# 87003697/DynamiCrafter

Hardware: AMD Instinct MI355X
Metric: frames/sec (and denoising-step ms), 16f@576x1024, DDIM 50 (higher is better)
Workload: dtype bf16; 1 GPU; inference_1024_v1.0.yaml: 1 clip/GPU, 16 frames, latent 72x128, DDIM 50 uniform_trailing eta=1, CFG 7.5 batched (cond+uncond), guidance_rescale 0.7, v-param+ZTSNR+dynamic rescale, hipGraph-captured step; clips_per_gpu=1, parallelism=dp1 over 1 distinct clips (no data-path collective), conditioning=local (1 rank), outputs_finite=True

## Files before the change

### dynamicrafter_amd/_hip.py

```python
import ctypes as C
import os
import threading

_HERE = os.path.dirname(os.path.abspath(__file__))
LIB_PATH = os.environ.get("DC_HIP_LIB") or os.path.join(_HERE, "csrc", "libdcrafter_hip.so")

DC_GEMM_OUT_F32 = 1
DC_GEMM_GEGLU = 2
DC_GEMM_GELU = 4


class DcGemmParams(C.Structure):
    _fields_ = [
        ("A", C.c_void_p), ("W", C.c_void_p), ("C", C.c_void_p), ("bias", C.c_void_p),
        ("rowvec", C.c_void_p), ("residual", C.c_void_p),
        ("lda", C.c_int), ("ldc", C.c_int), ("ldr", C.c_int), ("rowvec_ld", C.c_int),
        ("rows_per_vec", C.c_int),
        ("M", C.c_int), ("N", C.c_int), ("K", C.c_int), ("n_pad", C.c_int),
        ("mode", C.c_int), ("Cin", C.c_int),
        ("IH", C.c_int), ("IW", C.c_int), ("OH", C.c_int), ("OW", C.c_int),
        ("stride", C.c_int), ("pad", C.c_int), ("ups", C.c_int),
        ("T", C.c_int), ("HW", C.c_int),
        ("flags", C.c_int), ("alpha", C.c_float),
        ("workspace", C.c_void_p), ("workspace_bytes", C.c_longlong),
    ]


class DcDdimParams(C.Structure):
    _fields_ = [
        ("a_t", C.c_void_p), ("a_prev", C.c_void_p), ("sigma_t", C.c_void_p), ("sqrt_one_minus_at", C.c_void_p),
        ("sqrt_acp_t", C.c_void_p), ("sqrt_1macp_t", C.c_void_p), ("scale_ratio", C.c_void_p),
        ("step_index", C.c_void_p),
        ("index", C.c_int), ("v_param", C.c_int),
        ("cfg_scale", C.c_float), ("cfg_img", C.c_float), ("guidance_rescale", C.c_float),
        ("temperature", C.c_float),
        ("e_nchw", C.c_int), ("noise_step_stride", C.c_int64),
    ]


class DcDpmParams(C.Structure):
    _fields_ = [
        ("A", C.c_void_p), ("alpha_t", C.c_void_p), ("alpha_p_r", C.c_void_p), ("k", C.c_void_p), ("N", C.c_void_p),
        ("sqrt_one_minus_at", C.c_void_p), ("sqrt_acp_t", C.c_void_p), ("sqrt_1macp_t", C.c_void_p),
        ("scale_ratio", C.c_void_p), ("step_index", C.c_void_p),
        ("index", C.c_int), ("v_param", C.c_int),
        ("cfg_scale", C.c_float), ("cfg_img", C.c_float), ("guidance_rescale", C.c_float),
        ("temperature", C.c_float),
        ("e_nchw", C.c_int), ("noise_step_stride", C.c_int64), ("x0_hist", C.c_void_p),
    ]


class DcSdsParams(C.Structure):
    _fields_ = [
        ("c1", C.c_void_p), ("c2", C.c_void_p), ("w", C.c_void_p), ("step_size", C.c_void_p), ("bc2_sqrt", C.c_void_p),
        ("step_index", C.c_void_p), ("index", C.c_int), ("weight_type", C.c_int), ("x0_param", C.c_int),
        ("e_nchw", C.c_int), ("cfg_scale", C.c_float), ("guidance_rescale", C.c_float),
        ("beta2", C.c_float), ("eps", C.c_float), ("one_minus_beta1", C.c_float), ("one_minus_beta2", C.c_float),
        ("decay", C.c_float), ("grad_scale", C.c_float), ("noise_step_stride", C.c_int64), ("loss", C.c_void_p),
    ]


_P, _I, _F, _L = C.c_void_p, C.c_int, C.c_float, C.c_int64
SIGNATURES = {
    "dc_gemm_conv": (_I, [C.POINTER(DcGemmParams), _P]),
    "dc_gemm_workspace_bytes": (_L, []),
    "dc_gemm_last_variant": (C.c_char_p, []),
    "dc_gemm_set_plan": (_I, [_I]),
    "dc_groupnorm": (_I, [_P, _I, _P, _I, _P, _P, _I, _I, _I, _I, _F, _I, _P, _P]),
    "dc_groupnorm_workspace_bytes": (_L, [_I, _I, _I]),
    "dc_layernorm": (_I, [_P, _I, _P, _I, _P, _P, _I, _I, _F, _P]),
    "dc_flash_attn_d64": (_I, [_P, _P, _P, _P, _I, _I, _I, _I, _I, _I, _I, _I, _L, _L, _F, _I, _F, _P]),
    "dc_ff_geglu_fused320": (_I, [_P, _I, _P, _P, _F, _P, _P, _P, _P, _P, _I, _P, _I, _I, _P]),
    "dc_ff_geglu_proj_fused320": (_I, [_P, _I, _P, _P, _F, _P, _P, _P, _P, _P, _P, _P, _I, _P, _I, _I, _P]),
    "dc_ln_linear": (_I, [_P, _I, _I, _P, _P, _F, _P, _P, _P, _I, _I, _I, _P]),
    "dc_ln_qkv_temporal_attn320": (_I, [_P, _I, _P, _P, _F, _P, _P, _I, _I, _I, _I, _F, _P]),
    "dc_ln_qkv_temporal_attn640": (_I, [_P, _I, _P, _P, _F, _P, _P, _I, _I, _I, _I, _F, _P]),
    "dc_gn_silu_tconv3": (_I, [_P, _I, _I, _P, _P, _P, _I, _P, _P, _P, _I, _P, _I, _I, _I, _I, _I, _P]),
    "dc_groupnorm_stats": (_I, [_P, _I, _I, _I, _I, _I, _F, _P, _P, _P]),
    "dc_gn_linear": (_I, [_P, _I, _I, _P, _P, _P, _I, _I, _P, _P, _P, _I, _I, _I, _P]),
    "dc_flash_attn_set_mode": (_I, [_I, _F]),
    "dc_linear_residual": (_I, [_P, _I, _I, _P, _P, _P, _I, _P, _I, _I, _I, _P]),
    "dc_cross_attn_dual_d64": (_I, [_P, _P, _P, _P, _P, _P, _I, _I, _I, _I, _I, _I, _I, _I, _L, _L, _F, _F, _P]),
    "dc_temporal_attn_d64": (_I, [_P, _I, _P, _I, _I, _I, _I, _I, _F, _P]),
    "dc_gemv_small": (_I, [_P, _I, _P, _P, _P, _I, _I, _I, _I, _I, _I, _I, _P]),
    "dc_timestep_embedding": (_I, [_P, _P, _I, _P, _I, _I, _F, _P]),
    "dc_pack_latent": (_I, [_P, _P, _P, _I, _I, _I, _I, _I, _I, _I, _P]),
    "dc_nchw_to_rows": (_I, [_P, _P, _I, _I, _I, _I, _F, _P]),
    "dc_rows_to_nchw": (_I, [_P, _I, _I, _P, _I, _I, _I, _F, _P]),
    "dc_im2col3x3_c8": (_I, [_P, _I, _P, _I, _I, _I, _I, _P]),
    "dc_copy2d": (_I, [_P, _I, _P, _I, _I, _I, _P]),
    "dc_build_context": (_I, [_P, _P, _I, _I, _I, _I, _I, _P]),
    "dc_softmax_rows": (_I, [_P, _I, _P, _I, _I, _I, _P]),
    "dc_transpose": (_I, [_P, _I, _P, _I, _I, _I, _P]),
    "dc_add_rows": (_I, [_P, _I, _P, _I, _P, _I, _I, _I, _P]),
    "dc_vae_sample": (_I, [_P, _I, _P, _P, _I, _I, _I, _F, _P]),
    "dc_ddim_step": (_I, [C.POINTER(DcDdimParams), _P, _P, _P, _I, _P, _P, _P, _P, _I, _I, _I, _P, _P]),
    "dc_dpmpp_step": (_I, [C.POINTER(DcDpmParams), _P, _P, _P, _I, _P, _P, _P, _P, _I, _I, _I, _P, _P]),
    "dc_sds_noise": (_I, [C.POINTER(DcSdsParams), _P, _P, _P, _I, _L, _P]),
    "dc_sds_step": (_I, [C.POINTER(DcSdsParams), _P, _P, _I, _P, _P, _P, _P, _I, _I, _I, _P, _P]),
    "dc_attn_small": (_I, [_P, _P, _P, _P, _I, _I, _I, _I, _I, _I, _I, _I, _I, _F, _I, _P]),
    "dc_attn_small_lds_bytes": (_L, [_I, _I]),
    "dc_clip_preprocess": (_I, [_P, _P, _P, _P, _I, _I, _I, _I, _I, _I, _I, C.POINTER(_F), C.POINTER(_F), _P]),
    "dc_patchify": (_I, [_P, _P, _I, _I, _I, _I, _I, _I, _P]),
    "dc_embed_tokens": (_I, [_P, _P, _P, _P, _I, _I, _I, _I, _P]),
    "dc_frames_to_u8": (_I, [_P, _P, _I, _I, _I, _I, _I, _P]),
    "dc_mask_blend": (_I, [_P, _P, _P, _P, _P, _P, _P, _I, _L, _L, _I, _P]),
    "dc_advance_counter": (_I, [_P, _P]),
    "dc_stream_create": (_I, [C.POINTER(_P)]),
    "dc_stream_destroy": (_I, [_P]),
    "dc_stream_sync": (_I, [_P]),
    "dc_graph_begin_capture": (_I, [_P]),
    "dc_graph_end_capture": (_I, [_P, C.POINTER(_P)]),
    "dc_graph_launch": (_I, [_P, _P]),
    "dc_graph_destroy": (_I, [_P]),
    "dc_event_create": (_I, [C.POINTER(_P)]),
    "dc_event_record": (_I, [_P, _P]),
    "dc_event_elapsed_ms": (_I, [_P, _P, C.POINTER(_F)]),
    "dc_event_destroy": (_I, [_P]),
    "dc_error_word_read": (_I, [C.POINTER(C.c_int), _I]),
    "dc_version": (C.c_char_p, []),
}

_lib = None
_lock = threading.Lock()


def lib():
    global _lib
    if _lib is not None:
        return _lib
    with _lock:
        if _lib is None:
            if not os.path.exists(LIB_PATH):
                raise RuntimeError(
                    f"{LIB_PATH} not found: build it with dynamicrafter_amd/csrc/build.sh "
                    "(or __graft_entry__.build()); the HIP extension is mandatory, there is no fallback")
            import torch
            l = C.CDLL(LIB_PATH)
            for name, (res, args) in SIGNATURES.items():
                fn = getattr(l, name)
                fn.restype = res
                fn.argtypes = args
            _lib = l
    return _lib


ERROR_WORD_BITS = {1: "gemm_pipe320x16_kernel: LDS counter wait timed out",
                   2: "flash_attn_d64_pipe_kernel: K/V ring counter wait timed out",
                   4: "gemm_pp_kernel: LDS counter wait timed out"}


def check_error_word(what="", reset=True):
    w = C.c_int(0)
    check(lib().dc_error_word_read(C.byref(w), 1 if reset else 0), "dc_error_word_read")
    if w.value:
        names = [v for k, v in ERROR_WORD_BITS.items() if w.value & k] or [f"unknown bits {w.value:#x}"]
        raise RuntimeError(f"HIP kernels reported a failed wait ({what or 'error word'} = {w.value:#x}): " + "; ".join(names)
                           + " - results since the last check are NOT valid")


def check(code, what):
    if code != 0:
        raise RuntimeError(f"{what} failed with code {code}"
                           + (" (DC_ERR_SHAPE)" if code == -1 else " (DC_ERR_ARG)" if code == -2 else " (hipError_t)"))
```

### dynamicrafter_amd/csrc/gemm_conv.hip

```cpp
#include "dc_common.h"
#include "dcrafter_hip.h"
#include <stdlib.h>

namespace {

constexpr int BM = 128;
constexpr int BK = 64;
constexpr int NTHREADS = 256;

__device__ __forceinline__ int lds_off(int row, int chunk) {
    return row * 128 + ((chunk ^ ((row >> 1) & 7)) << 4);
}

__device__ __attribute__((aligned(16))) uint32_t g_zero_chunk[8];

template <int BN, bool GEGLU, int MODE>
__global__ __launch_bounds__(NTHREADS) void gemm_conv_kernel(const DcGemmParams p) {
    constexpr int NB = BN / 64;
    constexpr int BNOUT = GEGLU ? BN / 2 : BN;
    constexpr int A_BYTES = BM * BK * 2;
    constexpr int B_BYTES = BN * BK * 2;
    constexpr int STAGE = A_BYTES + B_BYTES;
    constexpr int B_ITERS = BN / 32;
    extern __shared__ __attribute__((aligned(16))) char smem[];
// ... 228 lines not shown
int launch_mode(const DcGemmParams& p, hipStream_t stream) {
    constexpr int BNOUT = GEGLU ? BN / 2 : BN;
    const int n_out = GEGLU ? p.N / 2 : p.N;
    const int tiles_n = (n_out + BNOUT - 1) / BNOUT;
    const int tiles_m = (p.M + BM - 1) / BM;
    const size_t lds = 2 * (BM * BK * 2 + BN * BK * 2);
    dc_note_variant(GEGLU ? "gemm_conv_kernel<geglu>" : (BN == 64 ? "gemm_conv_kernel<64>" : "gemm_conv_kernel<128>"));
    hipLaunchKernelGGL((gemm_conv_kernel<BN, GEGLU, MODE>), dim3(tiles_m * tiles_n), dim3(NTHREADS), lds, stream, p);
    DC_CHECK_LAUNCH();
    return 0;
}

template <int BN, bool GEGLU>
int launch(const DcGemmParams& p, hipStream_t stream) {
    if (p.mode == 0) return launch_mode<BN, GEGLU, 0>(p, stream);
    if (GEGLU) return DC_ERR_ARG;
    if (p.mode == 1) return launch_mode<BN, false, 1>(p, stream);
    if (p.mode == 2) return launch_mode<BN, false, 2>(p, stream);
    return DC_ERR_ARG;
}


constexpr int NC_TH = 4, NC_TW = 64;
constexpr int NC_WIN_W = NC_TW + 2, NC_WIN = (NC_TH + 2) * NC_WIN_W;
constexpr int NC_LDS = NC_WIN * 128;

__device__ __forceinline__ int nc_off(int px, int chunk) { return px * 128 + ((chunk ^ (px & 7)) << 4); }

template <bool F32>
__global__ __launch_bounds__(256) void conv3x3_narrow_kernel(const DcGemmParams p, const int tiles_x, const int tiles_y) {
    __shared__ __attribute__((aligned(16))) char win[NC_LDS];
    const int tid = threadIdx.x, lane = tid & 63;
    const int wave = __builtin_amdgcn_readfirstlane(tid >> 6);
    const int lj = lane & 15, lq = lane >> 4;
    const int per_frame = tiles_x * tiles_y;
    const int frame = (int)blockIdx.x / per_frame;
    const int trem = (int)blockIdx.x - frame * per_frame;
    const int ty0 = (trem / tiles_x) * NC_TH, tx0 = (trem % tiles_x) * NC_TW;
    const uint16_t* const fbase = p.A + (size_t)frame * p.IH * p.IW * p.lda;

    f32x4_t acc[NC_TW / 16];
#pragma unroll
    for (int b = 0; b < NC_TW / 16; ++b) acc[b] = f32x4_t{0.f, 0.f, 0.f, 0.f};

    const int nslices = p.Cin / 64;
    for (int sl = 0; sl < nslices; ++sl) {
        bf16x8_t wf[9][2];
        {
            const uint16_t* wrow = p.W + (size_t)lj * p.K + (size_t)sl * 576 + lq * 8;
#pragma unroll
            for (int t = 0; t < 9; ++t)
#pragma unroll
                for (int ks = 0; ks < 2; ++ks) {
                    u32x4_t v = {0u, 0u, 0u, 0u};
                    if (lj < p.N) v = *reinterpret_cast<const u32x4_t*>(wrow + t * 64 + ks * 32);
                    wf[t][ks] = __builtin_bit_cast(bf16x8_t, v);
                }
        }
        if (sl > 0) __syncthreads();
        constexpr int NC_IT = (NC_WIN * 8 + 255) / 256;
        u32x4_t stg[NC_IT];
#pragma unroll
        for (int it = 0; it < NC_IT; ++it) {
            int i = tid + it * 256;
            if (i >= NC_WIN * 8) i = NC_WIN * 8 - 1;
            const int px = i >> 3, ch = i & 7;
            const int wy = px / NC_WIN_W, wx = px - wy * NC_WIN_W;
            const int iy = ty0 + wy - 1, ix = tx0 + wx - 1;
            const bool in = iy >= 0 && iy < p.IH && ix >= 0 && ix < p.IW;
            const uint16_t* src = in ? fbase + ((size_t)iy * p.IW + ix) * p.lda + sl * 64 + ch * 8
                                     : reinterpret_cast<const uint16_t*>(g_zero_chunk);
            stg[it] = *reinterpret_cast<const u32x4_t*>(src);
        }
#pragma unroll
        for (int it = 0; it < NC_IT; ++it) {
            const int i = tid + it * 256;
            if (i < NC_WIN * 8) *reinterpret_cast<u32x4_t*>(win + nc_off(i >> 3, i & 7)) = stg[it];
        }
        __syncthreads();
#pragma unroll
        for (int t = 0; t < 9; ++t) {
            const int dy = t / 3, dx = t - 3 * dy;
#pragma unroll
            for (int ks = 0; ks < 2; ++ks)
#pragma unroll
                for (int b = 0; b < NC_TW / 16; ++b) {
                    const int px = (wave + dy) * NC_WIN_W + 16 * b + lj + dx;
                    const bf16x8_t xfrag = *reinterpret_cast<const bf16x8_t*>(win + nc_off(px, ks * 4 + lq));
                    acc[b] = __builtin_amdgcn_mfma_f32_16x16x32_bf16(wf[t][ks], xfrag, acc[b], 0, 0, 0);
                }
        }
    }
    const int oy = ty0 + wave;
    if (oy >= p.IH || 4 * lq >= p.N) return;
    float4 bv = make_float4(0.f, 0.f, 0.f, 0.f);
    if (p.bias) bv = *reinterpret_cast<const float4*>(p.bias + 4 * lq);
#pragma unroll
    for (int b = 0; b < NC_TW / 16; ++b) {
        const int ox = tx0 + 16 * b + lj;
        if (ox >= p.IW) continue;
        const size_t row = ((size_t)frame * p.IH + oy) * p.IW + ox;
        const float v0 = (acc[b][0] + bv.x) * p.alpha, v1 = (acc[b][1] + bv.y) * p.alpha;
        const float v2 = (acc[b][2] + bv.z) * p.alpha, v3 = (acc[b][3] + bv.w) * p.alpha;
        if constexpr (F32) {
            *reinterpret_cast<float4*>(reinterpret_cast<float*>(p.C) + row * p.ldc + 4 * lq) = make_float4(v0, v1, v2, v3);
        } else {
            uint2 pk;
            pk.x = pack_bf2(v0, v1); pk.y = pack_bf2(v2, v3);
            *reinterpret_cast<uint2*>(reinterpret_cast<uint16_t*>(p.C) + row * p.ldc + 4 * lq) = pk;
        }
    }
}

constexpr int WC_N = 128, WC_CB = WC_N / 16;
constexpr int WC_WST = WC_N * 128;
constexpr int NC_GROUPS = (NC_WIN + 7) / 8;
constexpr int WC_WIN_BYTES = NC_GROUPS * 1024;
constexpr int WC_LDS = WC_WIN_BYTES + WC_WST;

__global__ __launch_bounds__(256, 2) void conv3x3_window128_kernel(const DcGemmParams p, const int tiles_x, const int tiles_y) {
    extern __shared__ __attribute__((aligned(16))) char wsm[];
    char* const win = wsm;
    char* const wst = wsm + WC_WIN_BYTES;
    const unsigned lds_base = (unsigned)(uintptr_t)((const __attribute__((address_space(3))) char*)wsm);
    const int tid = threadIdx.x, lane = tid & 63;
    const int wave = __builtin_amdgcn_readfirstlane(tid >> 6);
    const int lj = lane & 15, lq = lane >> 4;
    const int per_frame = tiles_x * tiles_y;
    const int frame = (int)blockIdx.x / per_frame;
    const int trem = (int)blockIdx.x - frame * per_frame;
    const int ty0 = (trem / tiles_x) * NC_TH, tx0 = (trem % tiles_x) * NC_TW;
    const uint16_t* const fbase = p.A + (size_t)frame * p.IH * p.IW * p.lda;

    f32x4_t acc[NC_TW / 16][WC_CB];
#pragma unroll
    for (int b = 0; b < NC_TW / 16; ++b)
#pragma unroll
        for (int c = 0; c < WC_CB; ++c) acc[b][c] = f32x4_t{0.f, 0.f, 0.f, 0.f};

    u32x4_t wreg[4];
    auto w_fetch = [&](int sl, int t) __attribute__((always_inline)) {
#pragma unroll
        for (int i = 0; i < 4; ++i) {
            const int pc = tid + 256 * i;
            wreg[i] = *reinterpret_cast<const u32x4_t*>(p.W + (size_t)(pc >> 3) * p.K + (size_t)sl * 576 + t * 64 + (pc & 7) * 8);
        }
    };
    auto w_store = [&]() __attribute__((always_inline)) {
#pragma unroll
        for (int i = 0; i < 4; ++i) {
            const int pc = tid + 256 * i;
            *reinterpret_cast<u32x4_t*>(wst + nc_off(pc >> 3, pc & 7)) = wreg[i];
        }
    };

    const int nslices = p.Cin / 64;
    w_fetch(0, 0);
#pragma unroll 1
    for (int sl = 0; sl < nslices; ++sl) {
        if (sl > 0) __syncthreads();
        for (int g = wave; g < NC_GROUPS; g += 4) {
            const int px = g * 8 + (lane >> 3), ch = (lane & 7) ^ (px & 7);
            const int wy = px / NC_WIN_W, wx = px - wy * NC_WIN_W;
            const int iy = ty0 + wy - 1, ix = tx0 + wx - 1;
            const bool in = px < NC_WIN && iy >= 0 && iy < p.IH && ix >= 0 && ix < p.IW;
            const uint16_t* src = in ? fbase + ((size_t)iy * p.IW + ix) * p.lda + sl * 64 + ch * 8
                                     : reinterpret_cast<const uint16_t*>(g_zero_chunk);
            asm volatile("s_mov_b32 m0, %1\n\ts_nop 0\n\tglobal_load_lds_dwordx4 %0, off" ::"v"(src), "s"(lds_base + g * 1024) : "memory");
        }
        w_store();
        asm volatile("s_waitcnt vmcnt(0)" ::: "memory");
        __syncthreads();
#pragma unroll 1
        for (int t = 0; t < 9; ++t) {
            if (t + 1 < 9) w_fetch(sl, t + 1);
            else if (sl + 1 < nslices) w_fetch(sl + 1, 0);
            const int dy = t / 3, dx = t - 3 * dy;
#pragma unroll
            for (int ks = 0; ks < 2; ++ks) {
                bf16x8_t xb[NC_TW / 16];
#pragma unroll
                for (int b = 0; b < NC_TW / 16; ++b) {
                    const int px = (wave + dy) * NC_WIN_W + 16 * b + lj + dx;
                    xb[b] = *reinterpret_cast<const bf16x8_t*>(win + nc_off(px, ks * 4 + lq));
                }
#pragma unroll
                for (int c = 0; c < WC_CB; ++c) {
                    const bf16x8_t wa = *reinterpret_cast<const bf16x8_t*>(wst + nc_off(c * 16 + lj, ks * 4 + lq));
#pragma unroll
                    for (int b = 0; b < NC_TW / 16; ++b)
                        acc[b][c] = __builtin_amdgcn_mfma_f32_16x16x32_bf16(wa, xb[b], acc[b][c], 0, 0, 0);
                }
            }
            if (t + 1 < 9) {
                __syncthreads();
                w_store();
                __syncthreads();
            }
        }
    }
    __syncthreads();
    const int oy = ty0 + wave;
    if (oy >= p.IH) return;
    char* const patch = wsm + wave * 8192;
    uint16_t* const cbase = reinterpret_cast<uint16_t*>(p.C);
    const int rpx = lane >> 3, rch = lane & 7;
    const size_t row0 = ((size_t)frame * p.IH + oy) * p.IW + tx0;
#pragma unroll
    for (int hf = 0; hf < 2; ++hf) {
        u32x4_t rres[8];
        if (p.residual) {
#pragma unroll
            for (int it = 0; it < 8; ++it) {
                int px = it * 8 + rpx;
                if (tx0 + px >= p.IW) px = 0;
                rres[it] = *reinterpret_cast<const u32x4_t*>(p.residual + (row0 + px) * p.ldr + hf * 64 + rch * 8);
            }
        }
#pragma unroll
        for (int b = 0; b < NC_TW / 16; ++b)
#pragma unroll
            for (int c4 = 0; c4 < 4; ++c4) {
                const int c = hf * 4 + c4;
                float4 v = make_float4(acc[b][c][0], acc[b][c][1], acc[b][c][2], acc[b][c][3]);
                if (p.bias) {
                    const float4 bv = *reinterpret_cast<const float4*>(p.bias + 16 * c + 4 * lq);
                    v.x += bv.x; v.y += bv.y; v.z += bv.z; v.w += bv.w;
                }
                uint2 pk;
                pk.x = pack_bf2(v.x, v.y); pk.y = pack_bf2(v.z, v.w);
                const int px = 16 * b + lj;
                *reinterpret_cast<uint2*>(patch + nc_off(px, 2 * c4 + (lq >> 1)) + (lq & 1) * 8) = pk;
            }
#pragma unroll
        for (int it = 0; it < 8; ++it) {
            const int px = it * 8 + rpx;
            u32x4_t d = *reinterpret_cast<const u32x4_t*>(patch + nc_off(px, rch));
            if (p.residual) {
#pragma unroll
                for (int e = 0; e < 4; ++e)
                    d[e] = pack_bf2(__uint_as_float(d[e] << 16) + __uint_as_float(rres[it][e] << 16),
                                    __uint_as_float(d[e] & 0xffff0000u) + __uint_as_float(rres[it][e] & 0xffff0000u));
            }
            if (tx0 + px < p.IW) *reinterpret_cast<u32x4_t*>(cbase + (row0 + px) * p.ldc + hf * 64 + rch * 8) = d;
        }
    }
}

inline bool window128_conv_ok(const DcGemmParams& p) {
    if ((dc_gemm_plan_now() & 256) || p.mode != 1 || (p.N != WC_N && p.N != 2 * WC_N) || p.stride != 1 || p.pad != 1 || p.ups) return false;
    if (p.OH != p.IH || p.OW != p.IW || p.Cin % 64 != 0 || p.K != 9 * p.Cin || p.n_pad < p.N) return false;
    if (p.rowvec || p.flags || p.alpha != 1.0f) return false;
    if (p.M % (p.IH * p.IW) != 0 || ((uintptr_t)p.A % 16) != 0 || ((uintptr_t)p.W % 16) != 0 || ((uintptr_t)p.C % 8) != 0) return false;
    if (p.ldc % 8 != 0 || ((uintptr_t)p.C % 16) != 0 || (p.residual && (p.ldr % 8 != 0 || ((uintptr_t)p.residual % 16) != 0))) return false;
    const long long tiles = (long long)(p.M / (p.IH * p.IW)) * ((p.IW + NC_TW - 1) / NC_TW) * ((p.IH + NC_TH - 1) / NC_TH);
    return tiles >= 1024;
}

int launch_window128_conv(const DcGemmParams& p, hipStream_t stream) {
    static DcLdsOnce lds_once;
    if (const int e = lds_once.ensure(reinterpret_cast<const void*>(&conv3x3_window128_kernel), WC_LDS)) return e;
    const int tiles_x = (p.IW + NC_TW - 1) / NC_TW, tiles_y = (p.IH + NC_TH - 1) / NC_TH;
    const long long grid = (long long)(p.M / (p.IH * p.IW)) * tiles_x * tiles_y;
    if (grid <= 0 || grid > 0x7fffffffll) return DC_ERR_SHAPE;
    dc_note_variant(p.N == WC_N ? "conv3x3_window128_kernel" : "conv3x3_window128_kernel x2");
    for (int h = 0; h < p.N / WC_N; ++h) {
        DcGemmParams q = p;
        q.W = p.W + (size_t)h * WC_N * p.K;
        if (p.bias) q.bias = p.bias + h * WC_N;
        q.C = reinterpret_cast<uint16_t*>(p.C) + h * WC_N;
        if (p.residual) q.residual = p.residual + h * WC_N;
        q.N = WC_N;
        hipLaunchKernelGGL(conv3x3_window128_kernel, dim3((unsigned)grid), dim3(256), WC_LDS, stream, q, tiles_x, tiles_y);
        DC_CHECK_LAUNCH();
    }
    return 0;
}

inline bool narrow_conv_ok(const DcGemmParams& p) {
    if ((dc_gemm_plan_now() & 128) || p.mode != 1 || p.N > 16 || p.N % 4 != 0 || p.stride != 1 || p.pad != 1 || p.ups) return false;
    if (p.OH != p.IH || p.OW != p.IW || p.Cin % 64 != 0 || p.K != 9 * p.Cin) return false;
    if (p.residual || p.rowvec || (p.flags & ~DC_GEMM_OUT_F32)) return false;
    if (p.M % (p.IH * p.IW) != 0 || ((uintptr_t)p.A % 16) != 0 || ((uintptr_t)p.W % 16) != 0) return false;
    if ((p.flags & DC_GEMM_OUT_F32) ? ((uintptr_t)p.C % 16 != 0) : (((uintptr_t)p.C % 8) != 0)) return false;
    return true;
}

int launch_narrow_conv(const DcGemmParams& p, hipStream_t stream) {
    const int tiles_x = (p.IW + NC_TW - 1) / NC_TW, tiles_y = (p.IH + NC_TH - 1) / NC_TH;
    const long long grid = (long long)(p.M / (p.IH * p.IW)) * tiles_x * tiles_y;
    if (grid <= 0 || grid > 0x7fffffffll) return DC_ERR_SHAPE;
    dc_note_variant("conv3x3_narrow_kernel");
    if (p.flags & DC_GEMM_OUT_F32)
        hipLaunchKernelGGL(conv3x3_narrow_kernel<true>, dim3((unsigned)grid), dim3(256), 0, stream, p, tiles_x, tiles_y);
    else
        hipLaunchKernelGGL(conv3x3_narrow_kernel<false>, dim3((unsigned)grid), dim3(256), 0, stream, p, tiles_x, tiles_y);
    DC_CHECK_LAUNCH();
    return 0;
}

}

int dc_gemm_conv_glds_try(const DcGemmParams& p, hipStream_t stream);

static bool glds_enabled() {
    static int v = -1;
    if (v < 0) {
        const char* e = getenv("DC_GEMM_GLDS");
        v = (e && e[0] == '0') ? 0 : 1;
    }
    return v == 1;
}

static thread_local const char* g_last_variant = "none";
void dc_note_variant(const char* name) { g_last_variant = name; }
extern "C" const char* dc_gemm_last_variant(void) { return g_last_variant; }

extern "C" int64_t dc_gemm_workspace_bytes(void) {
    return (int64_t)8 * 40 * 256 * 320 * 4;
}

extern "C" int dc_gemm_conv(const DcGemmParams* pp, void* stream_) {
    const DcGemmParams& p = *pp;
    hipStream_t stream = (hipStream_t)stream_;
    if (p.M <= 0 || p.N <= 0 || p.K <= 0) return DC_ERR_SHAPE;
    if (p.K % BK != 0 || p.N % 4 != 0 || p.lda % 8 != 0 || p.ldc % 4 != 0) return DC_ERR_SHAPE;
    if (p.mode != 0 && (p.Cin % BK != 0)) return DC_ERR_SHAPE;
    if (p.mode == 1 && p.K != 9 * p.Cin) return DC_ERR_SHAPE;
    if (p.mode == 2 && p.K != 3 * p.Cin) return DC_ERR_SHAPE;
    if (p.residual && (p.ldr % 4 != 0)) return DC_ERR_SHAPE;
    const bool geglu = (p.flags & DC_GEMM_GEGLU) != 0;
    if (geglu && ((p.N / 2) % 64 != 0 || p.n_pad < p.N)) return DC_ERR_SHAPE;
    if (p.n_pad < (p.N + 127) / 128 * 128) return DC_ERR_SHAPE;
    if (narrow_conv_ok(p)) return launch_narrow_conv(p, stream);
    if (window128_conv_ok(p)) return launch_window128_conv(p, stream);
    if (glds_enabled()) {
        const int r = dc_gemm_conv_glds_try(p, stream);
        if (r != -100) return r;
    }
    if (geglu) return launch<128, true>(p, stream);
    const int t128 = (p.N + 127) / 128 * 128;
    const bool use64 = (p.N <= 64) || ((float)t128 / (float)p.N > 1.15f);
    if (use64) {
        if (p.n_pad < (p.N + 63) / 64 * 64) return DC_ERR_SHAPE;
        return launch<64, false>(p, stream);
    }
    if (p.n_pad < t128) return DC_ERR_SHAPE;
    return launch<128, false>(p, stream);
}
```

### dynamicrafter_amd/csrc/gemm_conv_glds.hip

```cpp
#include "dc_common.h"
#include "dcrafter_hip.h"
#include <stdint.h>
#include <stdlib.h>
#include <type_traits>
#include <utility>

namespace {

constexpr int GBM = 256;
constexpr int GBK = 64;
constexpr int GNT = 512;

typedef __attribute__((address_space(3))) char lds_char_t;

__device__ __attribute__((aligned(16))) uint32_t g_zero_chunk2[8];

__device__ __forceinline__ int lds_off2(int row, int chunk) {
    return row * 128 + ((chunk ^ ((row >> 1) & 7)) << 4);
}

__device__ __forceinline__ void glds16(const void* gsrc, unsigned lds_dst_uniform) {
    unsigned keep;
    asm volatile(
        "s_mov_b32 %0, m0\n\t"
// ... 526 lines not shown

    const unsigned lds_base = (unsigned)(unsigned long)((lds_char_t*)smem);
    const bf16_t* const zero_ptr = reinterpret_cast<const bf16_t*>(g_zero_chunk2);
    const int srow = lane >> 3;
    const int pchunk = lane & 7;

    const bf16_t* a_ptr[A_IT];
    int a_aux[A_IT];
    const bf16_t* b_ptr[B_IT];
    int i_tile = 0, i_kt = 0, i_stage = 0;
    int i_m0 = 0, i_n0 = 0;
    auto set_issue_tile = [&](int j) __attribute__((always_inline)) {
        const int logical = xcd_remap((int)blockIdx.x + j * G, ntiles);
        int tn, tmi;
        persist_tile(logical, tiles_m, tiles_n, tile_group, tmi, tn);
        const int m0 = tmi * GBM, n0 = tn * BNOUT;
        i_m0 = m0; i_n0 = n0;
#pragma unroll
        for (int q = 0; q < A_IT; ++q) {
            const int r = (q * 8 + wave) * 8 + srow;
            const int chunk = pchunk ^ ((r >> 1) & 7);
            const int m = m0 + r;
            const bool ok = m < p.M;
            a_aux[q] = 0;
            if (MODE == 0) {
                a_ptr[q] = ok ? p.A + (size_t)m * p.lda + chunk * 8 : nullptr;
            } else if (MODE == 1) {
                const int ohw = p.OH * p.OW;
                const int mm = ok ? m : 0;
                const int n = mm / ohw;
                const int rem = mm - n * ohw;
                const int oy = rem / p.OW;
                const int ox = rem - oy * p.OW;
                const int iy0 = oy * p.stride - p.pad, ix0 = ox * p.stride - p.pad;
                int mask = 0;
#pragma unroll
                for (int t = 0; t < 9; ++t) {
                    const int iy = iy0 + t / 3, ix = ix0 + t % 3;
                    if (ok && iy >= 0 && iy < p.IH && ix >= 0 && ix < p.IW) mask |= 1 << t;
                }
                a_aux[q] = mask;
                a_ptr[q] = p.A + ((long long)n * p.IH * p.IW + (long long)iy0 * p.IW + ix0) * p.lda + chunk * 8;
            } else {
                a_ptr[q] = p.A + (size_t)(ok ? m : 0) * p.lda + chunk * 8;
                a_aux[q] = ok ? (m / p.HW) % p.T : -1000;
            }
        }
#pragma unroll
        for (int q = 0; q < B_IT; ++q) {
            const int r = (q * 8 + wave) * 8 + srow;
            const int chunk = pchunk ^ ((r >> 1) & 7);
            int wrow;
            if (GEGLU) wrow = (r < BN / 2) ? (n0 + r) : ((p.N >> 1) + n0 + (r - BN / 2));
            else wrow = n0 + r;
            b_ptr[q] = p.W + (size_t)wrow * p.K + chunk * 8;
        }
    };
    auto issue_next_part = [&](int part) __attribute__((always_inline)) {
        const int k0 = i_kt * GBK;
        const unsigned sa = lds_base + i_stage * STAGE;
        const unsigned sb = sa + A_BYTES;
        const bool res_tile = RES_RING && i_kt >= nk;
#pragma unroll
        for (int q = 0; q < A_IT; ++q) {
            if (q != part) continue;
            const bf16_t* src;
            if (res_tile) {
                const int r = (q * 8 + wave) * 8 + srow;
                const int chunk = pchunk ^ ((r >> 1) & 7);
                const int m = i_m0 + r;
                const int col = i_n0 + (i_kt - nk) * 32 + (chunk >> 2) * (BN / 2) + (chunk & 3) * 8;
                src = (m < p.M) ? p.residual + (size_t)m * p.ldr + col : zero_ptr;
            } else if (MODE == 0) {
                src = a_ptr[q] ? a_ptr[q] + k0 : zero_ptr;
            } else if (MODE == 1) {
                const int cs = i_kt / 9;
                const int tap = i_kt - cs * 9;
                const int dy = tap / 3, dx = tap - dy * 3;
                const long long toff = (long long)(dy * p.IW + dx) * p.lda + cs * 64;
                src = ((a_aux[q] >> tap) & 1) ? a_ptr[q] + toff : zero_ptr;
            } else {
                const int cs = i_kt / 3;
                const int tap = i_kt - cs * 3;
                const long long shift = (long long)(tap - 1) * p.HW * p.lda + cs * 64;
                const int tt = a_aux[q] + tap - 1;
                src = (tt >= 0 && tt < p.T) ? a_ptr[q] + shift : zero_ptr;
            }
            glds16(src, sa + (q * 8 + wave) * 1024);
        }
        if (!res_tile) {
#pragma unroll
            for (int q = 0; q < B_IT; ++q)
                if ((q & 3) == part) glds16(b_ptr[q] + k0, sb + (q * 8 + wave) * 1024);
        }
        if (part == 3) {
            if (++i_stage >= GSTAGES) i_stage = 0;
            if (++i_kt >= nkr) {
                i_kt = 0;
                ++i_tile;
                if (i_tile < nj) set_issue_tile(i_tile);
            }
        }
    };
    auto issue_next = [&]() __attribute__((always_inline)) {
#pragma unroll
        for (int part = 0; part < 4; ++part) issue_next_part(part);
    };

    f32x16_t acc[2][NB];
    auto zero_acc = [&]() __attribute__((always_inline)) {
#pragma unroll
        for (int i = 0; i < 2; ++i)
#pragma unroll
            for (int j = 0; j < NB; ++j)
#pragma unroll
                for (int r = 0; r < 16; ++r) acc[i][j][r] = 0.f;
    };
    zero_acc();

    set_issue_tile(0);
    issue_next();
    if (GSTAGES >= 3 && total > 1) issue_next();
    if (GSTAGES == 4 && total > 2) issue_next();

    int c_tile = 0, c_kt = 0, stage = 0;
    for (int g = 0; g < total; ++g) {
        const int younger = total - 1 - g;
        if (GSTAGES == 4 && younger >= 2) {
            static_assert(GSTAGES != 4 || !RES_RING, "4-deep ring: residual tiles not counted");
            wait_vmcnt<2 * LOADS>();
        } else if (GSTAGES >= 3 && younger >= 1) {
            if (RES_RING && c_kt + 1 >= nk) wait_vmcnt<A_IT>(); else wait_vmcnt<LOADS>();
        } else {
            wait_vmcnt<0>();
        }
        __builtin_amdgcn_s_barrier();
        asm volatile("" ::: "memory");
        const bool more = g + GSTAGES - 1 < total;
        const char* sa = smem + stage * STAGE;
        const char* sb = sa + A_BYTES;
        {
#pragma unroll
            for (int kk = 0; kk < GBK / 16; ++kk) {
                if (more) issue_next_part(kk);
                bf16x8_t xf[2], wf[NB];
#pragma unroll
                for (int mb = 0; mb < 2; ++mb)
                    xf[mb] = *reinterpret_cast<const bf16x8_t*>(sa + lds_off2(wm * 64 + mb * 32 + fr, kk * 2 + fh));
#pragma unroll
                for (int nb = 0; nb < NB; ++nb) {
                    int brow;
                    if (GEGLU) brow = (nb < NBX ? 0 : BN / 2) + wn * (BN / 4) + (nb % NBX) * 32;
                    else brow = wn * (32 * NB) + nb * 32;
                    wf[nb] = *reinterpret_cast<const bf16x8_t*>(sb + lds_off2(brow + fr, kk * 2 + fh));
                }
#pragma unroll
                for (int mb = 0; mb < 2; ++mb)
#pragma unroll
                    for (int nb = 0; nb < NB; ++nb)
                        acc[mb][nb] = __builtin_amdgcn_mfma_f32_32x32x16_bf16(wf[nb], xf[mb], acc[mb][nb], 0, 0, 0);
            }
        }
        if (++stage >= GSTAGES) stage = 0;
        if (++c_kt >= nk) {
            if constexpr (RES_RING) {
#pragma unroll
                for (int j = 0; j < NB; ++j) {
                    ++g;
                    const int younger_r = total - 1 - g;
                    if (GSTAGES >= 3 && younger_r >= 1) {
                        if (j + 1 < NB) wait_vmcnt<A_IT>(); else wait_vmcnt<LOADS>();
                    } else {
                        wait_vmcnt<0>();
                    }
                    __builtin_amdgcn_s_barrier();
                    asm volatile("" ::: "memory");
                    if (g + GSTAGES - 1 < total) {
#pragma unroll
                        for (int kk = 0; kk < GBK / 16; ++kk) issue_next_part(kk);
                    }
                    const char* sr = smem + stage * STAGE;
                    int lane_r = lane;
                    asm volatile("" : "+v"(lane_r));
                    const int fr_r = lane_r & 31, fh_r = lane_r >> 5;
#pragma unroll
                    for (int i = 0; i < 2; ++i) {
                        const int e1 = fr_r - 16 * i - 8 * fh_r;
                        bf16x8_t idf;
#pragma unroll
                        for (int e = 0; e < 8; ++e) idf[e] = (e == e1) ? (short)0x3F80 : (short)0;
#pragma unroll
                        for (int mb = 0; mb < 2; ++mb) {
                            const bf16x8_t xr = *reinterpret_cast<const bf16x8_t*>(
                                sr + lds_off2(wm * 64 + mb * 32 + fr_r, (wn * 2 + i) * 2 + fh_r));
                            acc[mb][j] = __builtin_amdgcn_mfma_f32_32x32x16_bf16(idf, xr, acc[mb][j], 0, 0, 0);
                        }
                    }
                    if (++stage >= GSTAGES) stage = 0;
                }
            }
            c_kt = 0;
            const int logical = xcd_remap((int)blockIdx.x + c_tile * G, ntiles);
            ++c_tile;
            int tn, tmi;
            persist_tile(logical, tiles_m, tiles_n, tile_group, tmi, tn);
            const int m0 = tmi * GBM, n0 = tn * BNOUT;
            persist_epilogue<BN, GEGLU, EPI>(acc, p, m0, n0, n_out, wm, wn, lane, smem + GSTAGES * STAGE + wave * 2048);
            zero_acc();
        }
    }
}

template <int BN, bool GEGLU, int EPI, int MODE, int ST_FORCE>
int launch_persist_epi_st(const DcGemmParams& p, hipStream_t stream, int grid);

template <int BN, bool GEGLU, int EPI, int MODE>
int launch_persist_epi(const DcGemmParams& p, hipStream_t stream, int grid) {
    static const int st = [] { const char* e = getenv("DC_GEMM_STAGES"); return e ? atoi(e) : 0; }();
    if constexpr (BN <= 128 && MODE == 0 && !GEGLU) { if (st == 2) return launch_persist_epi_st<BN, GEGLU, EPI, MODE, 2>(p, stream, grid); }
    return launch_persist_epi_st<BN, GEGLU, EPI, MODE, 0>(p, stream, grid);
}

template <int BN, bool GEGLU, int EPI, int MODE, int ST_FORCE>
int launch_persist_epi_st(const DcGemmParams& p, hipStream_t stream, int grid) {
    constexpr int ST = ST_FORCE ? ST_FORCE : ((BN <= 128) ? 3 : 2);
    constexpr size_t lds = (size_t)ST * (GBM * GBK * 2 + BN * GBK * 2) + 8 * 2048;
    static_assert(lds <= 163840, "LDS budget");
    static DcLdsOnce lds_once;
    if (const int e = lds_once.ensure(reinterpret_cast<const void*>(&gemm_persist_kernel<BN, GEGLU, ST, EPI, MODE>), (int)lds)) return e;
    dc_note_variant(GEGLU ? (BN == 256 ? "gemm_persist_kernel<256,geglu>" : "gemm_persist_kernel<128,geglu>")
                    : MODE == 1 ? "gemm_persist_kernel<320,conv>" : MODE == 2 ? "gemm_persist_kernel<320,tconv>"
                    : BN == 320 ? (EPI == 1 || EPI == 3 ? "gemm_persist_kernel<320,residual>" : "gemm_persist_kernel<320>")
                    : BN == 128 ? "gemm_persist_kernel<128>" : "gemm_persist_kernel<64>");
    static const int group = [] { const char* e = getenv("DC_GEMM_GROUP"); return e ? atoi(e) : 8; }();
    hipLaunchKernelGGL((gemm_persist_kernel<BN, GEGLU, ST, EPI, MODE>), dim3(grid), dim3(GNT), lds, stream, p,
                       (group == 2 || group == 4 || group == 8 || group == 16) ? group : 1);
    DC_CHECK_LAUNCH();
    return 0;
}

inline bool ring_residual_ok(const DcGemmParams& p) {
    static const int on = [] { const char* e = getenv("DC_GEMM_RING_RESIDUAL"); return e ? atoi(e) : 1; }();
    return on && p.residual && !(p.flags & (DC_GEMM_GELU | DC_GEMM_GEGLU | DC_GEMM_OUT_F32)) && p.alpha == 1.0f &&
           (p.N % 64 == 0) && (p.ldr % 8 == 0) && ((uintptr_t)p.residual % 16 == 0);
}

template <int BN, bool GEGLU>
int launch_persist(const DcGemmParams& p, hipStream_t stream, int grid) {
    if (p.flags & DC_GEMM_OUT_F32) {
        if constexpr (GEGLU) return DC_ERR_ARG;
        else return launch_persist_epi<BN, GEGLU, 2, 0>(p, stream, grid);
    }
    if (p.residual) {
        if constexpr (!GEGLU) { if (ring_residual_ok(p) && p.N % BN == 0) return launch_persist_epi<BN, GEGLU, 3, 0>(p, stream, grid); }
        return launch_persist_epi<BN, GEGLU, 1, 0>(p, stream, grid);
    }
    return launch_persist_epi<BN, GEGLU, 0, 0>(p, stream, grid);
}

int launch_persist_conv320(const DcGemmParams& p, hipStream_t stream) {
    const bool ring = ring_residual_ok(p);
    if (p.mode == 1) return p.residual ? (ring ? launch_persist_epi<320, false, 3, 1>(p, stream, 256)
                                               : launch_persist_epi<320, false, 1, 1>(p, stream, 256))
                                       : launch_persist_epi<320, false, 0, 1>(p, stream, 256);
    return p.residual ? (ring ? launch_persist_epi<320, false, 3, 2>(p, stream, 256)
                              : launch_persist_epi<320, false, 1, 2>(p, stream, 256))
                      : launch_persist_epi<320, false, 0, 2>(p, stream, 256);
}

template <int BN, bool GEGLU, int MODE, int GSTAGES>
int launch_glds(const DcGemmParams& p, hipStream_t stream) {
    constexpr int BNOUT = GEGLU ? BN / 2 : BN;
    const int n_out = GEGLU ? p.N / 2 : p.N;
    const int tiles_n = (n_out + BNOUT - 1) / BNOUT;
    const int tiles_m = (p.M + GBM - 1) / GBM;
    constexpr size_t lds = (size_t)GSTAGES * (GBM * GBK * 2 + BN * GBK * 2);
    static DcLdsOnce lds_once;
    if (const int e = lds_once.ensure(reinterpret_cast<const void*>(&gemm_conv_glds_kernel<BN, GEGLU, MODE, GSTAGES>), (int)lds)) return e;
    GemmSplit sp;
    sp.partial = nullptr; sp.splits = 1; sp.tile_begin = 0; sp.tile_count = tiles_m * tiles_n; sp.err = nullptr; sp.whole = 0;
    dc_note_variant(GEGLU ? "gemm_conv_glds_kernel<geglu>"
                    : BN == 320 ? (MODE == 0 ? "gemm_conv_glds_kernel<320>" : MODE == 2 ? "gemm_conv_glds_kernel<320,tconv>" : "gemm_conv_glds_kernel<320,conv>")
                    : BN == 256 ? (MODE == 0 ? "gemm_conv_glds_kernel<256>" : MODE == 2 ? "gemm_conv_glds_kernel<256,tconv>" : "gemm_conv_glds_kernel<256,conv>")
                    : (MODE == 0 ? "gemm_conv_glds_kernel<128>" : MODE == 2 ? "gemm_conv_glds_kernel<128,tconv>" : "gemm_conv_glds_kernel<128,conv>"));
    hipLaunchKernelGGL((gemm_conv_glds_kernel<BN, GEGLU, MODE, GSTAGES>), dim3(tiles_m * tiles_n), dim3(GNT), lds, stream, p, sp);
    DC_CHECK_LAUNCH();
    return 0;
}

constexpr int PLAN_DEFAULT = 3 | 16;
constexpr int PLAN_MASK = 3 | 16 | 32 | 64 | 128 | 256;
inline bool plan_valid(int plan) { return plan >= 0 && plan <= 511 && !(plan & 4); }
std::atomic<int> g_gemm_plan{[] {
    const char* e = getenv("DC_GEMM_PLAN");
    const int v = e ? atoi(e) : PLAN_DEFAULT;
    return plan_valid(v) ? (v & PLAN_MASK) : PLAN_DEFAULT;
}()};
inline int pipe_min_k() { static const int v = [] { const char* e = getenv("DC_PIPE_MIN_K"); return e ? atoi(e) : 1920; }(); return v; }

template <int MODE, int EPI>
int launch_pipe_shape(const DcGemmParams& p, hipStream_t stream, GemmSplit sp, int gx, int gy) {
    sp.err = dc_error_word_device();
    if (!sp.err) return DC_ERR_ARG;
    return launch_pipe320x16<MODE, EPI>(p, stream, sp, gx, gy);
}

inline bool pipe_ok(const DcGemmParams& p, int plan) {
    if (!(plan & 3) || (!(plan & 2) && p.mode != 1)) return false;
    if (p.mode != 1 && p.K < pipe_min_k()) return false;
    if (p.flags & (DC_GEMM_GEGLU | DC_GEMM_OUT_F32)) return false;
    if (p.ups && !(p.mode == 1 && p.ups == 1 && p.stride == 1 && p.pad == 1 && p.OH == 2 * p.IH && p.OW == 2 * p.IW)) return false;
    if (p.N % 320 != 0 || p.n_pad < p.N || p.K % 64 != 0 || p.lda % 8 != 0 || ((uintptr_t)p.A % 16) != 0) return false;
    if (p.ldc % 8 != 0 || ((uintptr_t)p.C % 16) != 0 || (long long)p.M * p.ldc >= (1ll << 31)) return false;
    if (p.residual && (p.ldr % 8 != 0 || ((uintptr_t)p.residual % 16) != 0 || (long long)p.M * p.ldr >= (1ll << 31))) return false;
    long long rows = p.M, extra = 0;
    if (p.mode == 1) { if (p.Cin % 64 != 0 || p.K != 9 * p.Cin) return false; rows = (long long)(p.M / (p.OH * p.OW) + 1) * p.IH * p.IW; extra = 2ll * p.IW + 2; }
    else if (p.mode == 2) { if (p.Cin % 64 != 0 || p.K != 3 * p.Cin) return false; extra = 2ll * p.HW; }
    else if (p.mode != 0) return false;
    if ((rows + extra) * p.lda * 2 >= (1ll << 31)) return false;
    if (320ll * p.K * 2 >= (1ll << 31)) return false;
    return true;
}

int launch_pipe_whole(const DcGemmParams& p, hipStream_t stream) {
    const int ntiles = ((p.M + GBM - 1) / GBM) * (p.N / 320);
    GemmSplit sp;
    sp.partial = nullptr; sp.splits = 1; sp.tile_begin = 0; sp.tile_count = ntiles; sp.err = nullptr; sp.whole = 0;
    dc_note_variant(p.mode == 0 ? "gemm_pipe320x16_kernel" : p.mode == 2 ? "gemm_pipe320x16_kernel<tconv>"
                    : p.ups ? "gemm_pipe320x16_kernel<conv,ups>" : "gemm_pipe320x16_kernel<conv>");
    if (p.mode == 0) return p.residual ? launch_pipe_shape<0, 1>(p, stream, sp, ntiles, 1) : launch_pipe_shape<0, 0>(p, stream, sp, ntiles, 1);
    if (p.mode == 1 && p.ups) return p.residual ? launch_pipe_shape<3, 1>(p, stream, sp, ntiles, 1) : launch_pipe_shape<3, 0>(p, stream, sp, ntiles, 1);
    if (p.mode == 1) return p.residual ? launch_pipe_shape<1, 1>(p, stream, sp, ntiles, 1) : launch_pipe_shape<1, 0>(p, stream, sp, ntiles, 1);
    return p.residual ? launch_pipe_shape<2, 1>(p, stream, sp, ntiles, 1) : launch_pipe_shape<2, 0>(p, stream, sp, ntiles, 1);
}

template <int MODE, int BN = 320>
int launch_glds320_split(const DcGemmParams& p, hipStream_t stream, int ntiles, int full, int splits, bool use_pipe, bool merged) {
    constexpr int GSTAGES = 2;
    constexpr size_t lds = (size_t)GSTAGES * (GBM * GBK * 2 + BN * GBK * 2);
    static DcLdsOnce lds_once;
    if (const int e = lds_once.ensure(reinterpret_cast<const void*>(&gemm_conv_glds_kernel<BN, false, MODE, GSTAGES>), (int)lds)) return e;
    if constexpr (BN == 320) {
        if (use_pipe) {
            dc_note_variant(MODE == 0 ? "gemm_pipe320x16_kernel+splitk" : MODE == 2 ? "gemm_pipe320x16_kernel<tconv>+splitk"
                            : MODE == 3 ? "gemm_pipe320x16_kernel<conv,ups>+splitk" : "gemm_pipe320x16_kernel<conv>+splitk");
            GemmSplit sp;
            sp.err = nullptr; sp.whole = 0;
            if (full > 0 && merged && full % 8 == 0) {
                sp.partial = reinterpret_cast<float*>(p.workspace); sp.splits = splits; sp.tile_begin = full; sp.tile_count = ntiles - full;
                sp.whole = full;
                const int gx = full + sp.tile_count * splits;
                if (const int e = p.residual ? launch_pipe_shape<MODE, 1>(p, stream, sp, gx, 1) : launch_pipe_shape<MODE, 0>(p, stream, sp, gx, 1)) return e;
                sp.whole = 0;
            } else {
                if (full > 0) {
                    sp.partial = nullptr; sp.splits = 1; sp.tile_begin = 0; sp.tile_count = full;
                    if (const int e = p.residual ? launch_pipe_shape<MODE, 1>(p, stream, sp, full, 1) : launch_pipe_shape<MODE, 0>(p, stream, sp, full, 1)) return e;
                }
                sp.partial = reinterpret_cast<float*>(p.workspace); sp.splits = splits; sp.tile_begin = full; sp.tile_count = ntiles - full;
                if (const int e = launch_pipe_shape<MODE, 0>(p, stream, sp, sp.tile_count, splits)) return e;
            }
            hipLaunchKernelGGL((splitk_reduce_kernel<BN>), dim3((GBM * (BN / 4) + 255) / 256, sp.tile_count), dim3(256), 0, stream, p, sp);
            DC_CHECK_LAUNCH();
            return 0;
        }
    }
    if constexpr (BN == 320)
        dc_note_variant(MODE == 0 ? "gemm_conv_glds_kernel<320>+splitk" : MODE == 2 ? "gemm_conv_glds_kernel<320,tconv>+splitk" : "gemm_conv_glds_kernel<320,conv>+splitk");
    else
        dc_note_variant(MODE == 0 ? "gemm_conv_glds_kernel<256>+splitk" : MODE == 2 ? "gemm_conv_glds_kernel<256,tconv>+splitk" : "gemm_conv_glds_kernel<256,conv>+splitk");
    GemmSplit sp;
    sp.err = nullptr; sp.whole = 0;
    if (full > 0) {
        sp.partial = nullptr; sp.splits = 1; sp.tile_begin = 0; sp.tile_count = full;
        hipLaunchKernelGGL((gemm_conv_glds_kernel<BN, false, MODE, GSTAGES>), dim3(full), dim3(GNT), lds, stream, p, sp);
        DC_CHECK_LAUNCH();
    }
    sp.partial = reinterpret_cast<float*>(p.workspace); sp.splits = splits; sp.tile_begin = full; sp.tile_count = ntiles - full;
    hipLaunchKernelGGL((gemm_conv_glds_kernel<BN, false, MODE, GSTAGES>), dim3(sp.tile_count, splits), dim3(GNT), lds, stream, p, sp);
    DC_CHECK_LAUNCH();
    hipLaunchKernelGGL((splitk_reduce_kernel<BN>), dim3((GBM * (BN / 4) + 255) / 256, sp.tile_count), dim3(256), 0, stream, p, sp);
    DC_CHECK_LAUNCH();
    return 0;
}

template <int BN, int GSTAGES>
int launch_glds_mode(const DcGemmParams& p, hipStream_t stream) {
    if (p.mode == 0) return launch_glds<BN, false, 0, GSTAGES>(p, stream);
    if (p.mode == 1) return p.ups ? launch_glds<BN, false, 3, GSTAGES>(p, stream) : launch_glds<BN, false, 1, GSTAGES>(p, stream);
    return launch_glds<BN, false, 2, GSTAGES>(p, stream);
}

inline int persist_max_k() {
    static const int v = [] { const char* e = getenv("DC_GEMM_PERSIST_MAXK"); return e ? atoi(e) : 2560; }();
    return v;
}

inline float wave_eff(int wgs) { return (float)wgs / (float)(((wgs + 255) / 256) * 256); }

}

int dc_gemm_conv_glds_try(const DcGemmParams& p, hipStream_t stream) {
    const bool geglu = (p.flags & DC_GEMM_GEGLU) != 0;
    const int n_out = geglu ? p.N / 2 : p.N;
    const int tiles_m = (p.M + GBM - 1) / GBM;
    static const int force = [] { const char* e = getenv("DC_GEMM_TILE"); return e ? atoi(e) : 0; }();
    static const int persist = [] { const char* e = getenv("DC_GEMM_PERSIST"); return e ? atoi(e) : 1; }();
    if (geglu && p.mode != 0) return DC_ERR_ARG;
    const bool out_f32 = (p.flags & DC_GEMM_OUT_F32) != 0;
    const bool epi16 = out_f32 || ((n_out % 8 == 0) && (p.ldc % 8 == 0) && ((long long)p.M * p.ldc < (1ll << 31)) &&
                                   ((long long)p.M * p.ldr < (1ll << 31)) && ((uintptr_t)p.C % 16 == 0) &&
                                   (!p.residual || ((p.ldr % 8 == 0) && ((uintptr_t)p.residual % 16 == 0))));
    const int plan = g_gemm_plan.load(std::memory_order_relaxed);
    const bool use_pipe = pipe_ok(p, plan);
    const bool prefer_pipe = (force == 0) && use_pipe;
    if (persist && force == 0 && p.mode == 0 && epi16 && p.K <= persist_max_k() && !prefer_pipe) {
        static const int wide = [] { const char* e = getenv("DC_GEMM_PERSIST_WIDE"); return e ? atoi(e) : 1; }();
        if (geglu && (plan & 16) && ((plan & 32) || p.K <= 640) && pp_ok(p) && tiles_m * (n_out / 64) >= 1024) return launch_pp(p, stream);
        if (geglu) {
            if (wide && n_out % 128 == 0 && tiles_m * (n_out / 128) >= 512) return launch_persist<256, true>(p, stream, 256);
            const int nt = tiles_m * (n_out / 64);
            if (nt >= 512) return launch_persist<128, true>(p, stream, 256);
        } else {
            if (wide && p.N % 320 == 0 && p.n_pad >= p.N && tiles_m * (p.N / 320) >= 512)
                return launch_persist<320, false>(p, stream, 256);
            const int t128n = (p.N + 127) / 128;
            const float waste = (float)(t128n * 128) / (float)p.N;
            if (waste <= 1.15f && tiles_m * t128n >= 512) return launch_persist<128, false>(p, stream, 256);
            const int t64n = (p.N + 63) / 64;
            if (waste > 1.15f && tiles_m * t64n >= 512) return launch_persist<64, false>(p, stream, 256);
        }
    }
    static const int persist_conv_maxk = [] { const char* e = getenv("DC_GEMM_PERSIST_CONV_MAXK"); return e ? atoi(e) : 2880; }();
    if (persist && force == 0 && !prefer_pipe && !geglu && !out_f32 && epi16 && (p.mode == 2 || (p.mode == 1 && !p.ups)) &&
        p.N % 320 == 0 && p.n_pad >= p.N && tiles_m * (p.N / 320) >= (p.mode == 1 ? 1024 : 512) && p.K <= persist_conv_maxk)
        return launch_persist_conv320(p, stream);
    if (geglu) {
        const int w256 = (n_out % 128 == 0 && p.n_pad >= p.N) ? tiles_m * (n_out / 128) : 0;
        const int w128 = tiles_m * (n_out / 64);
        if ((force == 256 || (force == 0 && w256 >= 512 && wave_eff(w256) > 0.8f)) && w256 > 0)
            return launch_glds<256, true, 0, 2>(p, stream);
        if (w128 < 384) return -100;
        return launch_glds<128, true, 0, 3>(p, stream);
    }
    const int t128 = (p.N + 127) / 128;
    const bool n320 = (p.N % 320 == 0) && (p.n_pad >= p.N);
    const int w320 = n320 ? tiles_m * (p.N / 320) : 0;
    const int w128 = tiles_m * t128;
    const float waste128 = (float)(t128 * 128) / (float)p.N;
    const bool pipe_conv = use_pipe && p.mode == 1 && force == 0;
    float s320 = n320 ? (pipe_conv ? 1.4f : 1.25f) * wave_eff(w320) : 0.f;
    float s128 = wave_eff(w128) / waste128;
    if (w320 < (pipe_conv ? 128 : 200)) s320 = 0.f;
    if (w128 < 384) s128 = 0.f;
    static const int splitk = [] { const char* e = getenv("DC_GEMM_SPLITK"); return e ? atoi(e) : 1; }();
    if (splitk && force == 0 && n320 && p.workspace && p.n_pad >= p.N) {
        const int nk = p.K / GBK;
        int full = 0, splits = 0;
        if (w320 < 200 && w320 >= 8) {
            splits = 256 / w320;
            if (splits > 12) splits = 12;
            while (splits > 2 && nk / splits < 12) --splits;
        } else if (w320 > 256 && w320 <= 1280 && (w320 % 256) != 0 && (w320 % 256) <= 128) {
            full = (w320 / 256) * 256;
            splits = 256 / (w320 - full);
            if (splits > 8) splits = 8;
            while (splits > 2 && nk / splits < 8) --splits;
        }
        const size_t need = (size_t)splits * (size_t)(w320 - full) * GBM * 320 * sizeof(float);
        if (splits >= 2 && nk / splits >= (full ? 8 : 12) && need <= (size_t)p.workspace_bytes) {
            const bool merged = !(plan & 64);
            if (p.mode == 0) return launch_glds320_split<0>(p, stream, w320, full, splits, use_pipe, merged);
            if (p.mode == 1) return p.ups ? launch_glds320_split<3>(p, stream, w320, full, splits, use_pipe, merged)
                                          : launch_glds320_split<1>(p, stream, w320, full, splits, use_pipe, merged);
            return launch_glds320_split<2>(p, stream, w320, full, splits, use_pipe, merged);
        }
    }
    static const int splitk256 = [] { const char* e = getenv("DC_GEMM_SPLITK256"); return e ? atoi(e) : 1; }();
    if (splitk && splitk256 && force == 0 && !n320 && !out_f32 && p.workspace && p.N % 256 == 0 && p.n_pad >= p.N && (p.mode != 1 || !p.ups)) {
        const int w256s = tiles_m * (p.N / 256), nk = p.K / GBK;
        if (w256s > 256 && w256s <= 1280 && (w256s % 256) != 0 && (w256s % 256) <= 128) {
            const int full = (w256s / 256) * 256;
            int splits = 256 / (w256s - full);
            if (splits > 8) splits = 8;
            while (splits > 2 && nk / splits < 8) --splits;
            const size_t need = (size_t)splits * (size_t)(w256s - full) * GBM * 256 * sizeof(float);
            if (splits >= 2 && nk / splits >= 8 && need <= (size_t)p.workspace_bytes) {
                if (p.mode == 0) return launch_glds320_split<0, 256>(p, stream, w256s, full, splits, false, false);
                if (p.mode == 1) return launch_glds320_split<1, 256>(p, stream, w256s, full, splits, false, false);
                return launch_glds320_split<2, 256>(p, stream, w256s, full, splits, false, false);
            }
        }
    }
    if (force == 320 && n320) return use_pipe ? launch_pipe_whole(p, stream) : launch_glds_mode<320, 2>(p, stream);
    if (force == 128 && w128 > 0 && waste128 <= 1.15f) return launch_glds_mode<128, 3>(p, stream);
    if (force == 1) return -100;
    const int w256 = (!n320 && p.N % 256 == 0 && p.n_pad >= p.N) ? tiles_m * (p.N / 256) : 0;
    if ((force == 256 || force == 0) && w256 >= 200 && 1.2f * wave_eff(w256) >= s128) return launch_glds_mode<256, 2>(p, stream);
    if (s320 > 0.f && s320 >= s128) return use_pipe ? launch_pipe_whole(p, stream) : launch_glds_mode<320, 2>(p, stream);
    if (s128 > 0.f && waste128 <= 1.15f) return launch_glds_mode<128, 3>(p, stream);
    return -100;
}

int dc_gemm_plan_now() { return g_gemm_plan.load(std::memory_order_relaxed); }

extern "C" int dc_gemm_set_plan(int plan) {
    if (!plan_valid(plan)) return DC_ERR_ARG;
    return g_gemm_plan.exchange(plan & PLAN_MASK, std::memory_order_relaxed);
}
```

### dynamicrafter_amd/csrc/gemm_pipe16.h

```cpp
#pragma once

typedef __attribute__((ext_vector_type(4))) float gp_f32x4_t;

#define GP16_MFMA_A(d, w, x) asm volatile("v_mfma_f32_16x16x32_bf16 %0, %1, %2, %0" : "+a"(d) : "v"(w), "v"(x))
#define GP16_MFMA_V(d, w, x) asm volatile("v_mfma_f32_16x16x32_bf16 %0, %1, %2, %0" : "+v"(d) : "v"(w), "v"(x))

__device__ __forceinline__ void gp16_settle(gp_f32x4_t (&acc)[4][20]) {
#pragma unroll
    for (int rb = 0; rb < 4; ++rb)
        asm volatile("s_nop 7\n\ts_nop 7"
                     : "+a"(acc[rb][0]), "+a"(acc[rb][1]), "+a"(acc[rb][2]), "+a"(acc[rb][3]), "+a"(acc[rb][4]), "+a"(acc[rb][5]),
                       "+a"(acc[rb][6]), "+a"(acc[rb][7]), "+a"(acc[rb][8]), "+a"(acc[rb][9]), "+a"(acc[rb][10]), "+a"(acc[rb][11]),
                       "+a"(acc[rb][12]), "+a"(acc[rb][13]), "+a"(acc[rb][14]), "+a"(acc[rb][15]), "+v"(acc[rb][16]), "+v"(acc[rb][17]),
                       "+v"(acc[rb][18]), "+v"(acc[rb][19]));
    asm volatile("s_nop 7\n\ts_nop 7" ::: "memory");
}

template <int MODE, int EPI>
__global__ __launch_bounds__(256, 1) __attribute__((amdgpu_waves_per_eu(1, 1)))
void gemm_pipe320x16_kernel(const DcGemmParams p, const GemmSplit sp) {
    extern __shared__ __attribute__((aligned(16))) char smem[];
    const int tid = threadIdx.x, lane = tid & 63;
    const int wave = __builtin_amdgcn_readfirstlane(tid >> 6);
    const int lr = lane & 15, lq = lane >> 4;

    const int tiles_n = p.N / 320;
    int bx = blockIdx.x, by = blockIdx.y, tile_begin = sp.tile_begin, tile_count = sp.tile_count, nsplit = sp.splits;
    float* partial = sp.partial;
    if (sp.whole > 0) {
        if (bx < sp.whole) { tile_begin = 0; tile_count = sp.whole; nsplit = 1; partial = nullptr; by = 0; }
        else { bx -= sp.whole; by = bx / tile_count; bx -= by * tile_count; }
    }
    const int swz = tile_begin + xcd_remap(bx, tile_count);
    const int tile_n = swz % tiles_n;
    const int tile_m = swz / tiles_n;
    const int m0 = tile_m * GBM;
    const int n0 = tile_n * 320;

    const int nk_all = p.K / GBK;
    const int kt_lo = (int)(((long long)by * nk_all) / nsplit);
    const int kt_hi = (int)(((long long)(by + 1) * nk_all) / nsplit);
    const int nk = kt_hi - kt_lo;

    gp_lds_int_t* const cnt_landed = (gp_lds_int_t*)(smem + GP_CNT);
    gp_lds_int_t* const cnt_freed = cnt_landed + 1;
    if (tid < 2) cnt_landed[tid] = 0;
    __syncthreads();
    int gave_up = 0;

    const unsigned lda2 = (unsigned)p.lda * 2u;
    unsigned rowoff[4];
    int mask[4];
    long long bias = 0;
    if (MODE == 1) bias = (long long)(p.pad * p.IW + p.pad) * lda2;
    if (MODE == 2) bias = (long long)p.HW * lda2;
    if (MODE == 3) bias = (long long)(p.IW + 1) * lda2;
#ifdef GP_DBG_QUAD_ROWS
    const int lr_a = lr & ~3, lq_a = lane & 3;
#else
    const int lr_a = lr, lq_a = lq;
#endif
#pragma unroll
    for (int rb = 0; rb < 4; ++rb) {
        const int m = m0 + wave * 64 + rb * 16 + lr_a;
        const bool ok = m < p.M;
        const int mm = ok ? m : 0;
        if (MODE == 0) {
            rowoff[rb] = (unsigned)mm * lda2 + lq_a * 16;
            mask[rb] = ok ? 1 : 0;
        } else if (MODE == 1) {
            const int ohw = p.OH * p.OW;
            const int n = mm / ohw;
            const int rem = mm - n * ohw;
            const int oy = rem / p.OW;
            const int ox = rem - oy * p.OW;
            const int iy0 = oy * p.stride - p.pad, ix0 = ox * p.stride - p.pad;
            int mk = 0;
#pragma unroll
            for (int t = 0; t < 9; ++t) {
                const int iy = iy0 + t / 3, ix = ix0 + t % 3;
                if (ok && iy >= 0 && iy < p.IH && ix >= 0 && ix < p.IW) mk |= 1 << t;
            }
            mask[rb] = mk;
            rowoff[rb] = (unsigned)(((n * p.IH + iy0 + p.pad) * p.IW + ix0 + p.pad)) * lda2 + lq_a * 16;
        } else if (MODE == 3) {
            const int ohw = p.OH * p.OW;
            const int n = mm / ohw;
            const int rem = mm - n * ohw;
            const int oy = rem / p.OW;
            const int ox = rem - oy * p.OW;
            int mk = 0;
#pragma unroll
            for (int t = 0; t < 9; ++t) {
                const int uy = oy + t / 3 - 1, ux = ox + t % 3 - 1;
                if (ok && uy >= 0 && uy < p.OH && ux >= 0 && ux < p.OW) mk |= 1 << t;
            }
            mask[rb] = mk | ((oy & 1) << 9) | ((ox & 1) << 10);
            rowoff[rb] = (unsigned)(((n * p.IH + (oy >> 1) + 1) * p.IW + (ox >> 1) + 1)) * lda2 + lq_a * 16;
        } else {
            const int frame = (mm / p.HW) % p.T;
            int mk = 0;
#pragma unroll
            for (int t = 0; t < 3; ++t) {
                const int tt = frame + t - 1;
                if (ok && tt >= 0 && tt < p.T) mk |= 1 << t;
            }
            mask[rb] = mk;
            rowoff[rb] = (unsigned)mm * lda2 + lq_a * 16;
        }
    }
    gp_i32x4_t ars;
    {
        const unsigned long long ab = (unsigned long long)(uintptr_t)p.A - (unsigned long long)bias;
        ars[0] = __builtin_amdgcn_readfirstlane((int)(unsigned)ab);
        ars[1] = __builtin_amdgcn_readfirstlane((int)(unsigned)((ab >> 32) & 0xffffu));
        ars[2] = 0x7fffffff;
        ars[3] = 0x00020000;
    }
    auto a_tile = [&](int kt, unsigned (&vo)[4], int& soff) __attribute__((always_inline)) {
        int tap = 0;
        if (MODE == 0) {
            soff = kt * 128;
        } else if (MODE == 1) {
            const int cs = kt / 9;
            tap = kt - cs * 9;
            const int dy = tap / 3, dx = tap - dy * 3;
            soff = (dy * p.IW + dx) * (int)lda2 + cs * 128;
        } else if (MODE == 3) {
            const int cs = kt / 9;
            tap = kt - cs * 9;
            const int dy = tap / 3, dx = tap - dy * 3;
            soff = cs * 128;
            const int y0 = dy == 0 ? -p.IW * (int)lda2 : 0, y1 = dy == 2 ? p.IW * (int)lda2 : 0;
            const int x0 = dx == 0 ? -(int)lda2 : 0, x1 = dx == 2 ? (int)lda2 : 0;
#pragma unroll
            for (int rb = 0; rb < 4; ++rb) {
                const unsigned o = rowoff[rb] + (unsigned)(((mask[rb] >> 9) & 1) ? y1 : y0) + (unsigned)(((mask[rb] >> 10) & 1) ? x1 : x0);
                vo[rb] = ((mask[rb] >> tap) & 1) ? o : 0x80000000u;
            }
            return;
        } else {
            const int cs = kt / 3;
            tap = kt - cs * 3;
            soff = tap * p.HW * (int)lda2 + cs * 128;
        }
#pragma unroll
        for (int rb = 0; rb < 4; ++rb) vo[rb] = ((mask[rb] >> tap) & 1) ? rowoff[rb] : 0x80000000u;
    };

    const unsigned lds_base = (unsigned)(uintptr_t)((const __attribute__((address_space(3))) char*)smem);
    unsigned voffB[10];
#pragma unroll
    for (int j = 0; j < 10; ++j) {
        const int row = (j * 4 + wave) * 8 + (lane >> 3);
        voffB[j] = (unsigned)row * (unsigned)p.K * 2u + (unsigned)(((lane & 7) ^ (((wave & 1) * 4 + (lane >> 4)) & 7)) << 4);
        asm volatile("" : "+v"(voffB[j]));
    }
    auto w_src = [&](int kt) __attribute__((always_inline)) -> unsigned long long {
        return (unsigned long long)(uintptr_t)p.W + ((unsigned long long)n0 * p.K + (unsigned long long)kt * 64) * 2ull;
    };
    auto dma = [&](unsigned lds_dst, unsigned voff, unsigned long long sbase) __attribute__((always_inline)) {
        asm volatile("s_mov_b32 m0, %0\n\ts_nop 0\n\tglobal_load_lds_dwordx4 %1, %2" ::"s"(lds_dst), "v"(voff), "s"(sbase) : "memory");
    };

    unsigned bofs[3][2];
#pragma unroll
    for (int st = 0; st < 3; ++st)
#pragma unroll
        for (int s = 0; s < 2; ++s) {
            bofs[st][s] = lds_base + st * GP_STAGE + lr * 128 + (((4 * s + lq) ^ ((lr >> 1) & 7)) << 4);
            asm volatile("" : "+v"(bofs[st][s]));
        }
    bf16x8_t Bf[5];
    auto rd_b = [&](int slot, unsigned addr, int cb) __attribute__((always_inline)) {
        Bf[slot] = *(gp_lds_frag_t*)((const __attribute__((address_space(3))) char*)(uintptr_t)addr + cb * 2048);
    };

    u32x4_t A[3][4][2];
    gp_f32x4_t acc[4][20];
#pragma unroll
    for (int i = 0; i < 4; ++i)
#pragma unroll
        for (int j = 0; j < 20; ++j)
#pragma unroll
            for (int r = 0; r < 4; ++r) acc[i][j][r] = 0.f;

    auto clampk = [&](int t) { return kt_lo + (t < nk ? t : nk - 1); };
#pragma unroll
    for (int t = 0; t < 2; ++t) {
        const unsigned long long ws = w_src(clampk(t));
#pragma unroll
        for (int j = 0; j < 10; ++j) dma(lds_base + t * GP_STAGE + (j * 4 + wave) * 1024, voffB[j], ws);
        unsigned vo[4];
        int soff;
        a_tile(clampk(t), vo, soff);
#pragma unroll
        for (int i = 0; i < 8; ++i) {
            if ((i >> 2) == 0) GP_LOAD_A_(A[t][i & 3][0], vo[i & 3], ars, soff, "0");
            else GP_LOAD_A_(A[t][i & 3][1], vo[i & 3], ars, soff, "64");
        }
    }
    wait_vmcnt<26>();
    if (lane == 0) __hip_atomic_fetch_add(cnt_landed, 1, __ATOMIC_RELAXED, __HIP_MEMORY_SCOPE_WORKGROUP);
    {
        int seen = *(volatile gp_lds_int_t*)cnt_landed;
        GP_SPIN(__builtin_amdgcn_readfirstlane(seen) < 4, seen = *(volatile gp_lds_int_t*)cnt_landed);
        asm volatile("" ::: "memory");
    }
#pragma unroll
    for (int f = 0; f < 4; ++f) rd_b(f, bofs[0][0], f);
    gp16_settle(acc);

    int seen_f = 0, seen_l = 0;
    auto tile = [&](auto ST_, int t) __attribute__((always_inline)) {
        constexpr int ST = decltype(ST_)::value, ST1 = (ST + 1) % 3, ST2 = (ST + 2) % 3;
        const int kt2 = clampk(t + 2);
        unsigned vo[4] = {0u, 0u, 0u, 0u};
        int soff = 0;
        unsigned long long ws = 0;
        gp_f32x4_t (&acc1)[4][20] = acc;
        bf16x8_t (&Bf1)[5] = Bf;
        u32x4_t (&A1)[3][4][2] = A;
        gp_for(std::make_integer_sequence<int, 160>{}, [&](auto G_) __attribute__((always_inline)) {
            constexpr int g = decltype(G_)::value;
            gp_f32x4_t (&acc_)[4][20] = acc1;
            bf16x8_t (&Bf_)[5] = Bf1;
            u32x4_t (&A_)[3][4][2] = A1;
            if constexpr (g == 0) {
                wait_vmcnt<18>();
#pragma unroll
                for (int i = 0; i < 8; ++i) asm volatile("" : "+v"(A_[ST][i & 3][i >> 2]));
            }
            if constexpr ((g & 3) == 0) {
                constexpr int F = g / 4 + 4;
                if constexpr (F < 40) rd_b(F % 5, bofs[ST][F / 20], F % 20);
                else rd_b(F % 5, bofs[ST1][0], F - 40);
            } else if constexpr ((g & 3) == 2) {
                if constexpr (g == 2) seen_f = *(volatile gp_lds_int_t*)cnt_freed;
                if constexpr (g == 6) {
                    GP_SPIN(__builtin_amdgcn_readfirstlane(seen_f) < 4 * t, seen_f = *(volatile gp_lds_int_t*)cnt_freed);
                    asm volatile("" ::: "memory");
                    ws = w_src(kt2);
                }
                if constexpr (g >= 10 && g <= 82 && ((g - 10) & 7) == 0) {
                    constexpr int j = (g - 10) >> 3;
                    dma(lds_base + ST2 * GP_STAGE + (j * 4 + wave) * 1024, voffB[j], ws);
                }
                if constexpr (g == 86) {
                    wait_vmcnt<18>();
#ifdef GP_DBG_SKIP_POST
                    if (lane == 0 && !(wave == 3 && t == 1))
#else
                    if (lane == 0)
#endif
                        __hip_atomic_fetch_add(cnt_landed, 1, __ATOMIC_RELAXED, __HIP_MEMORY_SCOPE_WORKGROUP);
                    a_tile(kt2, vo, soff);
                }
                if constexpr (g >= 90 && g <= 146 && ((g - 90) & 7) == 0) {
                    constexpr int i = (g - 90) >> 3;
                    if constexpr ((i >> 2) == 0) GP_LOAD_A_(A_[ST2][i & 3][0], vo[i & 3], ars, soff, "0");
                    else GP_LOAD_A_(A_[ST2][i & 3][1], vo[i & 3], ars, soff, "64");
                }
                if constexpr (g == 118) seen_l = *(volatile gp_lds_int_t*)cnt_landed;
                if constexpr (g == 142) {
                    GP_SPIN(t + 1 < nk && __builtin_amdgcn_readfirstlane(seen_l) < 4 * (t + 2), seen_l = *(volatile gp_lds_int_t*)cnt_landed);
                    asm volatile("" ::: "memory");
                }
                if constexpr (g == 150) {
                    if (lane == 0) __hip_atomic_fetch_add(cnt_freed, 1, __ATOMIC_RELAXED, __HIP_MEMORY_SCOPE_WORKGROUP);
                }
            }
            constexpr int f = g / 4, rb = g & 3, s = f / 20, cb = f % 20;
            if constexpr (cb < 16) GP16_MFMA_A(acc_[rb][cb], Bf_[f % 5], A_[ST][rb][s]);
            else GP16_MFMA_V(acc_[rb][cb], Bf_[f % 5], A_[ST][rb][s]);
        });
    };
#ifdef GP_STAMPS
    const unsigned long long st_loop0 = __builtin_readcyclecounter();
    const unsigned long long st_real0 = __builtin_amdgcn_s_memrealtime();
#endif
    for (int t = 0; t < nk; t += 3) {
        tile(gp_ic<0>{}, t);
        if (t + 1 >= nk) break;
        tile(gp_ic<1>{}, t + 1);
        if (t + 2 >= nk) break;
        tile(gp_ic<2>{}, t + 2);
    }
    wait_vmcnt<0>();
    gp16_settle(acc);
    if (gave_up && lane == 0) atomicOr(sp.err, DC_ERRW_GEMM_PIPE);
#ifdef GP_STAMPS
    if (lane == 0 && p.workspace && !sp.partial && (size_t)(blockIdx.x * 4 + wave + 1) * 64 <= (size_t)p.workspace_bytes) {
        unsigned long long* out = reinterpret_cast<unsigned long long*>(p.workspace) + (size_t)(blockIdx.x * 4 + wave) * 8;
        out[0] = 0; out[1] = 0; out[2] = 0; out[3] = 0;
        out[4] = __builtin_readcyclecounter() - st_loop0; out[5] = (unsigned long long)nk;
        out[6] = __builtin_amdgcn_s_memrealtime() - st_real0;
    }
#endif

    if (partial) {
        const size_t slot = (size_t)by * tile_count + (size_t)(swz - tile_begin);
        float* const dst = partial + (slot * GBM + wave * 64 + lr) * 320 + 4 * lq;
#pragma unroll
        for (int rb = 0; rb < 4; ++rb)
#pragma unroll
            for (int cb = 0; cb < 20; ++cb)
                *reinterpret_cast<float4*>(dst + (size_t)rb * 16 * 320 + cb * 16) = make_float4(acc[rb][cb][0], acc[rb][cb][1], acc[rb][cb][2], acc[rb][cb][3]);
        return;
    }
    char* const ebuf = smem + GP_RING + wave * 2048;
    int lane_e = lane;
    asm volatile("" : "+v"(lane_e));
    const int er = lane_e & 15, eq = lane_e >> 4;
    const int rrow = lane_e >> 2, rc = lane_e & 3;
    const char* const rbase = reinterpret_cast<const char*>(p.residual);
    char* const cbase = reinterpret_cast<char*>(p.C);
#pragma unroll
    for (int rb = 0; rb < 4; ++rb) {
        const int m_acc = m0 + wave * 64 + rb * 16 + er;
        const float* rv = p.rowvec ? p.rowvec + (size_t)((m_acc < p.M ? m_acc : 0) / p.rows_per_vec) * p.rowvec_ld : nullptr;
        int mr = m0 + wave * 64 + rb * 16 + rrow;
        const bool rok = mr < p.M;
        if (!rok) mr = p.M - 1;
        const unsigned co = ((unsigned)mr * (unsigned)p.ldc + (unsigned)(n0 + rc * 8)) * 2u;
        const unsigned ro = ((unsigned)mr * (unsigned)p.ldr + (unsigned)(n0 + rc * 8)) * 2u;
#pragma unroll
        for (int cp = 0; cp < 10; ++cp) {
            u32x4_t rr;
            if constexpr (EPI == 1) rr = *reinterpret_cast<const u32x4_t*>(rbase + ro + cp * 64);
#pragma unroll
            for (int h = 0; h < 2; ++h) {
                const int cb = 2 * cp + h;
                const int n = n0 + cb * 16 + 4 * eq;
                float4 v = make_float4(acc[rb][cb][0], acc[rb][cb][1], acc[rb][cb][2], acc[rb][cb][3]);
                if (p.bias) {
                    const float4 bv = *reinterpret_cast<const float4*>(p.bias + n);
                    v.x += bv.x; v.y += bv.y; v.z += bv.z; v.w += bv.w;
                }
                if (p.flags & DC_GEMM_GELU) { v.x = DC_GELU(v.x); v.y = DC_GELU(v.y); v.z = DC_GELU(v.z); v.w = DC_GELU(v.w); }
                if (rv) {
                    const float4 r4 = *reinterpret_cast<const float4*>(rv + n);
                    v.x += r4.x; v.y += r4.y; v.z += r4.z; v.w += r4.w;
                }
                if (p.alpha != 1.0f) { v.x *= p.alpha; v.y *= p.alpha; v.z *= p.alpha; v.w *= p.alpha; }
                uint2 pk;
                pk.x = pack_bf2(v.x, v.y);
                pk.y = pack_bf2(v.z, v.w);
                *reinterpret_cast<uint2*>(ebuf + er * 64 + ((((4 * h + eq) ^ (((er >> 1) & 3) << 1))) << 3)) = pk;
            }
            u32x4_t d = *reinterpret_cast<const u32x4_t*>(ebuf + rrow * 64 + ((rc ^ ((rrow >> 1) & 3)) << 4));
            if constexpr (EPI == 1) {
#pragma unroll
                for (int e = 0; e < 4; ++e)
                    d[e] = pack_bf2(__uint_as_float(d[e] << 16) + __uint_as_float(rr[e] << 16),
                                    __uint_as_float(d[e] & 0xffff0000u) + __uint_as_float(rr[e] & 0xffff0000u));
            }
            if (rok) *reinterpret_cast<u32x4_t*>(cbase + co + cp * 64) = d;
            __builtin_amdgcn_sched_barrier(0);
        }
    }
}

template <int MODE, int EPI>
int launch_pipe320x16(const DcGemmParams& p, hipStream_t stream, const GemmSplit& sp, int grid_x, int grid_y) {
    static DcLdsOnce lds_once;
    if (const int e = lds_once.ensure(reinterpret_cast<const void*>(&gemm_pipe320x16_kernel<MODE, EPI>), GP_LDS)) return e;
    hipLaunchKernelGGL((gemm_pipe320x16_kernel<MODE, EPI>), dim3(grid_x, grid_y), dim3(256), GP_LDS, stream, p, sp);
    DC_CHECK_LAUNCH();
    return 0;
}
```

### dynamicrafter_amd/lvdm/modules/networks/openaimodel3d.py

```python
import math

import torch
import torch.nn as nn

from .... import ops
from ....ops import PackedWeight
from ....param_tree import attach_params

import os

_BF16 = torch.bfloat16
_FF_FUSED = os.environ.get("DC_FF_FUSED", "1") != "0"
_LN_FUSED = os.environ.get("DC_LN_FUSED", "1") != "0"
_LR_FUSED = os.environ.get("DC_LR_FUSED", "1") != "0"
_TA_FUSED = os.environ.get("DC_TA_FUSED", "1") != "0"
_TA_FUSED_C = tuple(int(k) for k in os.environ.get("DC_TA_FUSED_C", "320,640").split(","))
_FFP_FUSED = os.environ.get("DC_FFP_FUSED", "1") != "0"
_TC_FUSED = os.environ.get("DC_TC_FUSED", "1") != "0"
_FUSED_MIN_ROWS = int(os.environ.get("DC_FUSED_MIN_ROWS", "4096"))
_LN_FUSED_K = tuple(int(k) for k in os.environ.get("DC_LN_FUSED_K", "320,640").split(","))
C_IN_PAD = 64


def _block_layout(cfg):
    mc, mults, nrb = cfg["model_channels"], list(cfg["channel_mult"]), cfg["num_res_blocks"]
    attn_res = set(cfg["attention_resolutions"])
    hc = cfg["num_head_channels"]
    tconv = bool(cfg["temporal_conv"])

    def transformers(ch):
        out = [("spatial", {"ch": ch, "heads": ch // hc})]
        if cfg["temporal_attention"]:
            out.append(("temporal", {"ch": ch, "inner": ch, "heads": ch // hc, "linear": bool(cfg["use_linear"])}))
        return out

    down_path = [[("conv_in", {"cin": cfg["in_channels"], "cout": mc})]]
    widths = [mc]
    ch, ds = mc, 1
    for lvl, m in enumerate(mults):
        for _ in range(nrb):
            blk = [("res", {"cin": ch, "cout": m * mc, "tconv": tconv})]
            ch = m * mc
            if ds in attn_res:
                blk += transformers(ch)
            down_path.append(blk)
            widths.append(ch)
        if lvl + 1 < len(mults):
            down_path.append([("down", {"ch": ch})])
            widths.append(ch)
            ds *= 2
    middle = [("res", {"cin": ch, "cout": ch, "tconv": tconv})] + transformers(ch) + \
             [("res", {"cin": ch, "cout": ch, "tconv": tconv})]
    up_path = []
    for lvl in reversed(range(len(mults))):
        for i in range(nrb + 1):
            skip = widths.pop()
            blk = [("res", {"cin": ch + skip, "cout": mults[lvl] * mc, "tconv": tconv})]
            ch = mults[lvl] * mc
            if ds in attn_res:
                blk += transformers(ch)
            if lvl and i == nrb:
                blk.append(("up", {"ch": ch}))
                ds //= 2
            up_path.append(blk)
    return down_path, middle, up_path


def _shape_table(cfg):
    t = {}
    mc = cfg["model_channels"]
    emb_dim = 4 * mc

    def affine(p, c):
        t[p + ".weight"] = (c,)
        t[p + ".bias"] = (c,)

    def dense(p, i, o, bias=True):
        t[p + ".weight"] = (o, i)
        if bias:
            t[p + ".bias"] = (o,)

    def conv(p, i, o, *k):
        t[p + ".weight"] = (o, i) + tuple(k)
        t[p + ".bias"] = (o,)

    def attn(p, dim, ctx, with_ip):
        dense(p + ".to_q", dim, dim, False)
        dense(p + ".to_k", ctx, dim, False)
        dense(p + ".to_v", ctx, dim, False)
        dense(p + ".to_out.0", dim, dim)
        if with_ip:
            dense(p + ".to_k_ip", ctx, dim, False)
            dense(p + ".to_v_ip", ctx, dim, False)
            if cfg["image_cross_attention_scale_learnable"]:
                t[p + ".alpha"] = ()

    def tblock(p, dim, ctx, with_ip):
        attn(p + ".attn1", dim, dim, False)
        dense(p + ".ff.net.0.proj", dim, 8 * dim)
        dense(p + ".ff.net.2", 4 * dim, dim)
        attn(p + ".attn2", dim, ctx, with_ip)
        for n in ("norm1", "norm2", "norm3"):
            affine(f"{p}.{n}", dim)

    def temporal(p, ch, inner, linear):
        affine(p + ".norm", ch)
        if linear:
            dense(p + ".proj_in", ch, inner)
        else:
            conv(p + ".proj_in", ch, inner, 1)
        tblock(p + ".transformer_blocks.0", inner, inner, False)
        if linear:
            dense(p + ".proj_out", inner, ch)
        else:
            conv(p + ".proj_out", inner, ch, 1)

    dense("time_embed.0", mc, emb_dim)
    dense("time_embed.2", emb_dim, emb_dim)
    if cfg["fs_condition"]:
        dense("fps_embedding.0", mc, emb_dim)
        dense("fps_embedding.2", emb_dim, emb_dim)

    def emit(prefix, blk):
        for j, (kind, a) in enumerate(blk):
            p = f"{prefix}.{j}"
            if kind == "conv_in":
                conv(p, a["cin"], a["cout"], 3, 3)
            elif kind == "res":
                affine(p + ".in_layers.0", a["cin"])
                conv(p + ".in_layers.2", a["cin"], a["cout"], 3, 3)
                dense(p + ".emb_layers.1", emb_dim, a["cout"])
                affine(p + ".out_layers.0", a["cout"])
                conv(p + ".out_layers.3", a["cout"], a["cout"], 3, 3)
                if a["cin"] != a["cout"]:
                    conv(p + ".skip_connection", a["cin"], a["cout"], 1, 1)
                if a["tconv"]:
                    for i, ci in ((1, 2), (2, 3), (3, 3), (4, 3)):
                        affine(f"{p}.temopral_conv.conv{i}.0", a["cout"])
                        conv(f"{p}.temopral_conv.conv{i}.{ci}", a["cout"], a["cout"], 3, 1, 1)
            elif kind == "spatial":
                affine(p + ".norm", a["ch"])
                dense(p + ".proj_in", a["ch"], a["ch"])
                tblock(p + ".transformer_blocks.0", a["ch"], cfg["context_dim"], bool(cfg["image_cross_attention"]))
                dense(p + ".proj_out", a["ch"], a["ch"])
            elif kind == "temporal":
                temporal(p, a["ch"], a["inner"], a["linear"])
            elif kind == "down":
                conv(p + ".op", a["ch"], a["ch"], 3, 3)
            elif kind == "up":
                conv(p + ".conv", a["ch"], a["ch"], 3, 3)

    down_path, middle, up_path = _block_layout(cfg)
    emit("input_blocks.0", down_path[0])
    if cfg["addition_attention"]:
        temporal("init_attn.0", mc, 8 * cfg["num_head_channels"], False)
    for i, blk in enumerate(down_path[1:], start=1):
        emit(f"input_blocks.{i}", blk)
    emit("middle_block", middle)
    for i, blk in enumerate(up_path):
        emit(f"output_blocks.{i}", blk)
    affine("out.0", mc)
    conv("out.2", mc, cfg["out_channels"], 3, 3)
    return t


_Arena = ops.Arena


class UNetModel(nn.Module):
    def __init__(self, in_channels, model_channels, out_channels, num_res_blocks, attention_resolutions,
                 dropout=0.0, channel_mult=(1, 2, 4, 8), conv_resample=True, dims=2, context_dim=None,
                 use_scale_shift_norm=False, resblock_updown=False, num_heads=-1, num_head_channels=-1,
                 transformer_depth=1, use_linear=False, use_checkpoint=False, temporal_conv=False,
                 tempspatial_aware=False, temporal_attention=True, use_relative_position=True,
                 use_causal_attention=False, temporal_length=None, use_fp16=False, addition_attention=False,
                 temporal_selfatt_only=True, image_cross_attention=False,
                 image_cross_attention_scale_learnable=False, default_fs=4, fs_condition=False):
        super().__init__()
        unsupported = []
        if dims != 2: unsupported.append("dims != 2")
        if use_scale_shift_norm: unsupported.append("use_scale_shift_norm")
        if resblock_updown: unsupported.append("resblock_updown")
        if not conv_resample: unsupported.append("conv_resample=False")
        if num_head_channels != 64: unsupported.append("num_head_channels != 64 (kernels are head_dim 64)")
        if transformer_depth != 1: unsupported.append("transformer_depth != 1")
        if not use_linear: unsupported.append("use_linear=False")
        if tempspatial_aware: unsupported.append("tempspatial_aware")
        if use_relative_position: unsupported.append("use_relative_position")
        if use_causal_attention: unsupported.append("use_causal_attention")
        if not temporal_selfatt_only: unsupported.append("temporal cross-attention")
        if context_dim is None: unsupported.append("context_dim=None")
        if temporal_length is not None and temporal_length > 16: unsupported.append("temporal_length > 16")
        if model_channels % 64 != 0: unsupported.append("model_channels % 64 != 0")
        if unsupported:
            raise NotImplementedError("UNetModel (HIP path) covers the released DynamiCrafter configurations; "
                                      "unsupported here: " + ", ".join(unsupported))
        self.in_channels, self.model_channels, self.out_channels = in_channels, model_channels, out_channels
        self.num_res_blocks = num_res_blocks
        self.attention_resolutions = list(attention_resolutions)
        self.channel_mult = list(channel_mult)
        self.dropout, self.use_checkpoint = dropout, use_checkpoint
        self.temporal_attention, self.temporal_length = temporal_attention, temporal_length
        self.addition_attention = addition_attention
        self.image_cross_attention = image_cross_attention
        self.image_cross_attention_scale_learnable = image_cross_attention_scale_learnable
        self.default_fs, self.fs_condition = default_fs, fs_condition
        self.context_dim = context_dim
        self.dtype = torch.float32
        self._cfg = dict(in_channels=in_channels, out_channels=out_channels, model_channels=model_channels,
                         attention_resolutions=list(attention_resolutions), num_res_blocks=num_res_blocks,
                         channel_mult=list(channel_mult), num_head_channels=num_head_channels,
                         context_dim=context_dim, temporal_conv=temporal_conv, temporal_attention=temporal_attention,
                         addition_attention=addition_attention, image_cross_attention=image_cross_attention,
                         image_cross_attention_scale_learnable=image_cross_attention_scale_learnable,
                         fs_condition=fs_condition, use_linear=use_linear)
        self._layout = _block_layout(self._cfg)
        self._cat_plan = self._make_cat_plan()
        attach_params(self, _shape_table(self._cfg))
        self._packed = None
        self._arena = _Arena()
        self.register_load_state_dict_post_hook(lambda m, k: setattr(m, "_packed", None))

    def _make_cat_plan(self):
        down_path, middle, up_path = self._layout
        out_ch = lambda blk: [a.get("cout", a.get("ch")) for k, a in blk if k in ("conv_in", "res", "down", "up")][-1]
        widths = [out_ch(b) for b in down_path]
        ch = out_ch(middle)
        plan = []
        for blk in up_path:
            skip = widths.pop()
            assert blk[0][1]["cin"] == ch + skip
            plan.append((ch, skip))
            ch = out_ch(blk)
        return plan

    def _p(self, name):
        node = self
        parts = name.split(".")
        for s in parts[:-1]:
            node = node._modules[s]
        return node._parameters[parts[-1]]

    def _has(self, name):
        node = self
        parts = name.split(".")
        for s in parts[:-1]:
            node = node._modules.get(s)
            if node is None:
                return False
        return parts[-1] in node._parameters

    def invalidate_packed(self):
        self._packed = None

    def _pack(self, device):
        P = {}
        f32 = lambda n: self._p(n).detach().to(device=device, dtype=torch.float32).contiguous()
        lin = lambda n: PackedWeight.linear(self._p(n + ".weight"), self._p(n + ".bias") if self._has(n + ".bias") else None, device)

        def attn_self(p):
            w = torch.cat([self._p(f"{p}.to_{x}.weight") for x in "qkv"], dim=0)
            return {"qkv": PackedWeight.linear(w, None, device), "out": lin(p + ".to_out.0")}

        def tblock(p, cross):
            d = {"attn1": attn_self(p + ".attn1"), "ff1": lin(p + ".ff.net.0.proj"), "ff2": lin(p + ".ff.net.2")}
            if d["ff2"].N == 320 and d["ff1"].N == 2560:
                d["ff2p"] = ops.ff2_permuted(self._p(p + ".ff.net.2.weight"), device)
            for n in ("norm1", "norm2", "norm3"):
                d[n] = (f32(f"{p}.{n}.weight"), f32(f"{p}.{n}.bias"))
            if cross:
                a = p + ".attn2"
                d["q2"] = lin(a + ".to_q")
                names = ["to_k", "to_v"] + (["to_k_ip", "to_v_ip"] if self.image_cross_attention else [])
                d["kv_ctx"] = PackedWeight.linear(torch.cat([self._p(f"{a}.{x}.weight") for x in names], 0), None, device)
                d["out2"] = lin(a + ".to_out.0")
                d["ip_scale"] = 1.0
                if self.image_cross_attention and self.image_cross_attention_scale_learnable:
                    d["ip_scale"] = float(torch.tanh(self._p(a + ".alpha").detach().float()).item() + 1.0)
            else:
                d["attn2"] = attn_self(p + ".attn2")
            d["key"] = p
            return d

        def with_projp(d, p):
            w = self._p(p + ".proj_out.weight")
            if "ff2p" in d["blk"] and w.shape[0] == 320 and w[0].numel() == 320:
                d["proj_p"] = ops.ff2_permuted(w.reshape(320, 320), device)
            return d

        def temporal(p):
            return with_projp({"norm": (f32(p + ".norm.weight"), f32(p + ".norm.bias")), "proj_in": lin(p + ".proj_in"),
                               "blk": tblock(p + ".transformer_blocks.0", False), "proj_out": lin(p + ".proj_out")}, p)

        P["time0"], P["time2"] = lin("time_embed.0"), lin("time_embed.2")
        if self.fs_condition:
            P["fps0"], P["fps2"] = lin("fps_embedding.0"), lin("fps_embedding.2")
        if self.addition_attention:
            P["init_attn"] = temporal("init_attn.0")

        def pack_block(prefix, blk):
            out = []
            for j, (kind, a) in enumerate(blk):
                p = f"{prefix}.{j}"
                if kind == "conv_in":
                    d = {"conv": PackedWeight.conv3x3(self._p(p + ".weight"), self._p(p + ".bias"), device)}
                    if a["cin"] <= 8 and os.environ.get("DC_CONVIN_IM2COL", "1") != "0":
                        d["lin8"] = PackedWeight.conv3x3_c8_as_linear(self._p(p + ".weight"), self._p(p + ".bias"), device)
                    out.append(d)
                elif kind == "res":
                    d = {"gn1": (f32(p + ".in_layers.0.weight"), f32(p + ".in_layers.0.bias")),
                         "conv1": PackedWeight.conv3x3(self._p(p + ".in_layers.2.weight"), self._p(p + ".in_layers.2.bias"), device),
                         "emb": lin(p + ".emb_layers.1"),
                         "gn2": (f32(p + ".out_layers.0.weight"), f32(p + ".out_layers.0.bias")),
                         "conv2": PackedWeight.conv3x3(self._p(p + ".out_layers.3.weight"), self._p(p + ".out_layers.3.bias"), device)}
                    if a["cin"] != a["cout"]:
                        d["skip"] = lin(p + ".skip_connection")
                    if a["tconv"]:
                        d["tc"] = []
                        for i, ci in ((1, 2), (2, 3), (3, 3), (4, 3)):
                            q = f"{p}.temopral_conv.conv{i}"
                            d["tc"].append(((f32(q + ".0.weight"), f32(q + ".0.bias")),
                                            PackedWeight.tconv3(self._p(f"{q}.{ci}.weight"), self._p(f"{q}.{ci}.bias"), device)))
                    out.append(d)
                elif kind == "spatial":
                    out.append(with_projp({"norm": (f32(p + ".norm.weight"), f32(p + ".norm.bias")), "proj_in": lin(p + ".proj_in"),
                                           "blk": tblock(p + ".transformer_blocks.0", True), "proj_out": lin(p + ".proj_out")}, p))
                elif kind == "temporal":
                    out.append(temporal(p))
                elif kind == "down":
                    out.append({"conv": PackedWeight.conv3x3(self._p(p + ".op.weight"), self._p(p + ".op.bias"), device)})
                elif kind == "up":
                    out.append({"conv": PackedWeight.conv3x3(self._p(p + ".conv.weight"), self._p(p + ".conv.bias"), device)})
            return out

        down_path, middle, up_path = self._layout
        P["in"] = [pack_block(f"input_blocks.{i}", b) for i, b in enumerate(down_path)]
        P["mid"] = pack_block("middle_block", middle)
        P["out"] = [pack_block(f"output_blocks.{i}", b) for i, b in enumerate(up_path)]
        P["out_gn"] = (f32("out.0.weight"), f32("out.0.bias"))
        P["out_conv"] = PackedWeight.conv3x3(self._p("out.2.weight"), self._p("out.2.bias"), device, n_align=4)
        P["device"] = device
        self._pack_gen = getattr(self, "_pack_gen", 0) + 1
        P["gen"] = self._pack_gen
        return P

    def packed(self, device):
        if self._packed is None or self._packed["device"] != device:
            self._packed = self._pack(device)
        return self._packed

    def _gn(self, x, wb, tag, *, n_inst, rpi, eps, silu):
        y = self._arena.get(tag, x.shape[0], x.shape[1], device=x.device)
        return ops.groupnorm(x, y, wb[0], wb[1], groups=32, n_inst=n_inst, rows_per_inst=rpi, eps=eps, silu=silu)

    def _ln(self, x, wb, tag):
        y = self._arena.get(tag, x.shape[0], x.shape[1], device=x.device)
        return ops.layernorm(x, y, wb[0], wb[1], 1e-5)

    def _res(self, W, x, g, out_tag, out=None):
        A = self._arena
        M, dev = x.shape[0], x.device
        cout = W["conv1"].N
        conv = dict(IH=g["H"], IW=g["W"], OH=g["H"], OW=g["W"], stride=1, pad=1, ups=0)
        emb_out = A.get("emb_out", g["B"], cout, torch.float32, dev)
        ops.gemv_small(g["emb"], W["emb"], emb_out, act_in=1)
        h = self._gn(x, W["gn1"], "gn", n_inst=g["F"], rpi=g["HW"], eps=1e-5, silu=True)
        h1 = ops.gemm(h, W["conv1"], A.get("res_h1", M, cout, device=dev), conv=conv, rowvec=emb_out,
                      rows_per_vec=g["T"] * g["HW"])
        h = self._gn(h1, W["gn2"], "gn", n_inst=g["F"], rpi=g["HW"], eps=1e-5, silu=True)
        skip = x
        if "skip" in W:
            skip = ops.gemm(x, W["skip"], A.get("res_skip", M, cout, device=dev))
        has_tc = "tc" in W
        final = (lambda: out if out is not None else A.get(out_tag, M, cout, device=dev))
        h2 = ops.gemm(h, W["conv2"], A.get("res_h2", M, cout, device=dev) if has_tc else final(), conv=conv,
                      residual=skip)
        if not has_tc:
            return h2
        tc = dict(T=g["T"], HW=g["HW"])
        r = h2
        fused_tc = (_TC_FUSED and cout in _LN_FUSED_K and g["T"] == 16 and g["HW"] % 8 == 0 and M >= _FUSED_MIN_ROWS
                    and (g["T"] * g["HW"]) % 128 == 0)
        for i, (gnw, cw) in enumerate(W["tc"]):
            last = i == 3
            dst = final() if last else A.get("res_ta" if i % 2 == 0 else "res_tb", M, cout, device=dev)
            if fused_tc:
                st = A.get("gn_stats", g["B"] * 32 * 2, 1, torch.float32, dev)
                ops.groupnorm_stats(r, st, groups=32, n_inst=g["B"], rows_per_inst=g["T"] * g["HW"], eps=1e-5)
                r = ops.gn_silu_tconv3(r, gnw[0], gnw[1], st, cw, dst, B=g["B"], T=16, HW=g["HW"],
                                           residual=h2 if last else None)
                continue
            n = self._gn(r, gnw, "gn", n_inst=g["B"], rpi=g["T"] * g["HW"], eps=1e-5, silu=True)
            r = ops.gemm(n, cw, dst, tconv=tc, residual=h2 if last else None)
        return r

    def _ln_linear(self, h, ln, pw, out):
        if _LN_FUSED and pw.K in _LN_FUSED_K and pw.N % 32 == 0 and h.shape[0] >= _FUSED_MIN_ROWS:
            return ops.ln_linear(h, pw, out, ln=ln, ln_eps=1e-5)
        return ops.gemm(self._ln(h, ln, "ln"), pw, out)

    def _lin_res(self, x, pw, res, out):
        if _LR_FUSED and pw.K in _LN_FUSED_K and pw.N % 32 == 0 and x.shape[0] >= _FUSED_MIN_ROWS:
            return ops.linear_residual(x, pw, res, out)
        return ops.gemm(x, pw, out, residual=res)

    def _gn_linear(self, x, gnw, pw, out, *, n_inst, rpi):
        if _LN_FUSED and pw.K in _LN_FUSED_K and pw.N % 32 == 0 and x.shape[0] >= _FUSED_MIN_ROWS and rpi % 128 == 0:
            st = self._arena.get("gn_stats", n_inst * 32 * 2, 1, torch.float32, x.device)
            ops.groupnorm_stats(x, st, groups=32, n_inst=n_inst, rows_per_inst=rpi, eps=1e-6)
            return ops.gn_linear(x, gnw[0], gnw[1], st, pw, out, groups=32, rows_per_inst=rpi)
        return ops.gemm(self._gn(x, gnw, "gn", n_inst=n_inst, rpi=rpi, eps=1e-6, silu=False), pw, out)

    def _attn_self_spatial(self, Wa, ln, h, g, heads):
        A = self._arena
        M, dev, Cc = h.shape[0], h.device, heads * 64
        qkv = self._ln_linear(h, ln, Wa["qkv"], A.get("qkv", M, 3 * Cc, device=dev))
        att = A.get("att", M, Cc, device=dev)
        ops.flash_attn(qkv[:, :Cc], qkv[:, Cc:2 * Cc], qkv[:, 2 * Cc:], att, batch=g["F"], heads=heads, Lq=g["HW"],
                       Lk=g["HW"], scale=0.125)
        return self._lin_res(att, Wa["out"], h, h)

    def _attn_self_temporal(self, Wa, ln, h, g, heads):
        A = self._arena
        M, dev, Cc = h.shape[0], h.device, heads * 64
        att = A.get("att", M, Cc, device=dev)
        if _TA_FUSED and Cc in _TA_FUSED_C and g["T"] == 16 and g["HW"] % 8 == 0 and M >= _FUSED_MIN_ROWS:
            ops.ln_qkv_temporal_attn(h, ln, Wa["qkv"], att, B=g["B"], T=16, HW=g["HW"], scale=0.125)
            return self._lin_res(att, Wa["out"], h, h)
        qkv = self._ln_linear(h, ln, Wa["qkv"], A.get("qkv", M, 3 * Cc, device=dev))
        ops.temporal_attn(qkv, att, B=g["B"], T=g["T"], HW=g["HW"], heads=heads, scale=0.125)
        return self._lin_res(att, Wa["out"], h, h)

    def _ff(self, Wb, h, tag="ln"):
        A = self._arena
        if "ff2p" in Wb and _FF_FUSED and h.shape[0] >= _FUSED_MIN_ROWS:
            return ops.ff_geglu_fused320(h, Wb["ff1"], Wb["ff2p"], Wb["ff2"].bias, h, residual=h, ln=Wb["norm3"], ln_eps=1e-5)
        n = self._ln(h, Wb["norm3"], tag)
        mid = ops.gemm(n, Wb["ff1"], A.get("ffmid", h.shape[0], Wb["ff1"].N // 2, device=h.device), geglu=True)
        return ops.gemm(mid, Wb["ff2"], h, residual=h)

    def _ff_proj(self, W, h, x, out):
        B_ = W["blk"]
        if "proj_p" in W and _FF_FUSED and _FFP_FUSED and h.shape[0] >= _FUSED_MIN_ROWS:
            return ops.ff_geglu_proj_fused320(h, B_["ff1"], B_["ff2p"], B_["ff2"].bias, W["proj_p"], W["proj_out"].bias, x, out,
                                              ln=B_["norm3"], ln_eps=1e-5)
        h = self._ff(B_, h)
        return self._lin_res(h, W["proj_out"], x, out)

    def _spatial_pre(self, W, x, g, heads):
        A = self._arena
        M, dev, Cc = x.shape[0], x.device, x.shape[1]
        h = self._gn_linear(x, W["norm"], W["proj_in"], A.get("tr_h", M, Cc, device=dev), n_inst=g["F"], rpi=g["HW"])
        B_ = W["blk"]
        return self._attn_self_spatial(B_["attn1"], B_["norm1"], h, g, heads)

    def _context_kv(self, B_, ctx, tag):
        return ops.gemm(ctx, B_["kv_ctx"], self._arena.get(tag, ctx.shape[0], B_["kv_ctx"].N, device=ctx.device))

    def precompute_context_kv(self, ctx_rows):
        Wt = self.packed(ctx_rows.device)
        down_path, middle, up_path = self._layout
        out = {"__gen__": Wt["gen"]}
        for name, blks, Ws in (("in", down_path, Wt["in"]), ("mid", [middle], [Wt["mid"]]), ("out", up_path, Wt["out"])):
            for i, (blk, Wb) in enumerate(zip(blks, Ws)):
                for j, ((kind, a), W) in enumerate(zip(blk, Wb)):
                    if kind == "spatial":
                        out[W["blk"]["key"]] = self._context_kv(W["blk"], ctx_rows, f"kvctx.{name}{i}.{j}")
        return out

    def _spatial_post(self, W, x, h, g, heads, out_tag, out=None):
        A = self._arena
        M, dev, Cc = x.shape[0], x.device, x.shape[1]
        B_ = W["blk"]
        q = self._ln_linear(h, B_["norm2"], B_["q2"], A.get("q2", M, Cc, device=dev))
        kv = None if g.get("ctx_kv") is None else g["ctx_kv"].get(B_["key"])
        if kv is None:
            kv = self._context_kv(B_, g["ctx"], "kvctx")
        att = A.get("att", M, Cc, device=dev)
        Lc, nt = g["Lc"], g["n_text"]
        if self.image_cross_attention and Lc > nt:
            ops.cross_attn_dual(q, kv[:, :Cc], kv[:, Cc:2 * Cc], kv[nt:, 2 * Cc:3 * Cc], kv[nt:, 3 * Cc:], att, batch=g["F"],
                                heads=heads, Lq=g["HW"], Lk=nt, Lk2=Lc - nt, scale=0.125, scale2=B_["ip_scale"], kv_bstride=Lc)
        else:
            ops.flash_attn(q, kv[:, :Cc], kv[:, Cc:2 * Cc], att, batch=g["F"], heads=heads, Lq=g["HW"], Lk=nt, scale=0.125,
                           kv_bstride=Lc)
        h = self._lin_res(att, B_["out2"], h, h)
        return self._ff_proj(W, h, x, out if out is not None else A.get(out_tag, M, Cc, device=dev))

    def _spatial(self, W, x, g, heads, out_tag, out=None):
        return self._spatial_post(W, x, self._spatial_pre(W, x, g, heads), g, heads, out_tag, out=out)

    def _temporal(self, W, x, g, heads, out_tag, out=None):
        A = self._arena
        M, dev, Cc = x.shape[0], x.device, x.shape[1]
        inner = W["proj_in"].N
        h = self._gn_linear(x, W["norm"], W["proj_in"], A.get("tr_h", M, inner, device=dev), n_inst=g["B"],
                            rpi=g["T"] * g["HW"])
        B_ = W["blk"]
        h = self._attn_self_temporal(B_["attn1"], B_["norm1"], h, g, heads)
        h = self._attn_self_temporal(B_["attn2"], B_["norm2"], h, g, heads)
        return self._ff_proj(W, h, x, out if out is not None else A.get(out_tag, M, Cc, device=dev))

    def _run_block(self, blk, Wb, h, g, tag, final=None):
        A = self._arena
        for j, ((kind, a), W) in enumerate(zip(blk, Wb)):
            out_tag = f"{tag}.{j}"
            dev = h.device
            last = final is not None and j == len(blk) - 1
            if kind == "conv_in":
                conv = dict(IH=g["H"], IW=g["W"], OH=g["H"], OW=g["W"], stride=1, pad=1, ups=0)
                dst = final(h.shape[0], a["cout"]) if last else A.get(out_tag, h.shape[0], a["cout"], device=dev)
                if "lin8" in W:
                    cols = ops.im2col3x3_c8(h, A.get(out_tag + ".im2col", h.shape[0], 128, device=dev), n_img=h.shape[0] // (g["H"] * g["W"]),
                                            H=g["H"], W=g["W"])
                    h = ops.gemm(cols, W["lin8"], dst)
                else:
                    h = ops.gemm(h, W["conv"], dst, conv=conv)
            elif kind == "res":
                h = self._res(W, h, g, out_tag, out=final(h.shape[0], a["cout"]) if last else None)
            elif kind == "spatial":
                h = self._spatial(W, h, g, a["heads"], out_tag, out=final(h.shape[0], a["ch"]) if last else None)
            elif kind == "temporal":
                h = self._temporal(W, h, g, a["heads"], out_tag, out=final(h.shape[0], a["ch"]) if last else None)
            elif kind == "down":
                OH, OW = (g["H"] + 1) // 2, (g["W"] + 1) // 2
                conv = dict(IH=g["H"], IW=g["W"], OH=OH, OW=OW, stride=2, pad=1, ups=0)
                rows = g["F"] * OH * OW
                h = ops.gemm(h, W["conv"], final(rows, a["ch"]) if last else A.get(out_tag, rows, a["ch"], device=dev), conv=conv)
                g["H"], g["W"], g["HW"] = OH, OW, OH * OW
            elif kind == "up":
                OH, OW = g["H"] * 2, g["W"] * 2
                conv = dict(IH=g["H"], IW=g["W"], OH=OH, OW=OW, stride=1, pad=1, ups=1)
                rows = g["F"] * OH * OW
                h = ops.gemm(h, W["conv"], final(rows, a["ch"]) if last else A.get(out_tag, rows, a["ch"], device=dev), conv=conv)
                g["H"], g["W"], g["HW"] = OH, OW, OH * OW
        return h

    def _replicate(self, src, tag, nrep, dst=None):
        if dst is None:
            dst = self._arena.get(tag, nrep * src.shape[0], src.shape[1], device=src.device)
        for k in range(nrep):
            ops.copy2d(src, dst[k * src.shape[0]:(k + 1) * src.shape[0]])
        return dst

    def forward_rows(self, xrows, t_table, ctx_rows, *, B, T, H, W, Lc, n_text=77, fs_table=None, t_index=None,
                     shared_prefix=1, ctx_kv=None):
        dev = xrows.device
        Wt = self.packed(dev)
        A = self._arena
        mc = self.model_channels
        temb = A.get("t_sin", B, mc, torch.float32, dev)
        ops.timestep_embedding(t_table, temb, mc, t_index=t_index, t_stride=B)
        hid = A.get("emb_hid", B, 4 * mc, torch.float32, dev)
        emb = A.get("emb", B, 4 * mc, torch.float32, dev)
        ops.gemv_small(temb, Wt["time0"], hid, act_out=1)
        ops.gemv_small(hid, Wt["time2"], emb)
        if self.fs_condition:
            femb = A.get("fs_sin", B, mc, torch.float32, dev)
            ops.timestep_embedding(fs_table, femb, mc)
            ops.gemv_small(femb, Wt["fps0"], hid, act_out=1)
            ops.gemv_small(hid, Wt["fps2"], emb, accumulate=True)
        if ctx_kv is not None and ctx_kv.get("__gen__") != Wt["gen"]:
            ctx_kv = None
        g = dict(B=B, T=T, F=B * T, H=H, W=W, HW=H * W, emb=emb, ctx=ctx_rows, Lc=Lc, n_text=n_text, ctx_kv=ctx_kv)
        down_path, middle, up_path = self._layout
        n_up = len(up_path)

        cat_rows = {}

        def cat_view(u, rows, part):
            ch, cs = self._cat_plan[u]
            if cat_rows.setdefault(u, rows) != rows:
                raise ValueError("skip / decoder resolution mismatch (the latent height and width must divide by 8)")
            buf = A.get(f"cat{u}", rows, ch + cs, device=dev)
            return buf[:, :ch] if part == "h" else buf[:, ch:]

        def skip_dst(d):
            return lambda rows, cols: cat_view(n_up - 1 - d, rows, "skip")

        h = xrows
        first = 0
        nrep = shared_prefix
        if nrep > 1 and len(down_path) > 1 and [k for k, _ in down_path[1]][:2] == ["res", "spatial"]:
            B1 = B // nrep
            g1 = dict(g, B=B1, F=B1 * T, emb=emb[:B1])
            h = self._run_block(down_path[0], Wt["in"][0], h[:B1 * T * H * W], g1, "in0")
            if self.addition_attention:
                h = self._temporal(Wt["init_attn"], h, g1, 8, "init_attn")
            self._replicate(h, None, nrep, dst=skip_dst(0)(nrep * h.shape[0], h.shape[1]))
            blk, Wb = down_path[1], Wt["in"][1]
            r = self._res(Wb[0], h, g1, "in1.0")
            hh = self._spatial_pre(Wb[1], r, g1, blk[1][1]["heads"])
            r_full = self._replicate(r, "in1.0.rep", nrep)
            h_full = self._replicate(hh, "tr_h.rep", nrep)
            last = len(blk) - 1
            fin = skip_dst(1)
            h = self._spatial_post(Wb[1], r_full, h_full, g, blk[1][1]["heads"], "in1.1",
                                   out=fin(r_full.shape[0], r_full.shape[1]) if last == 1 else None)
            for j in range(2, len(blk)):
                kind, a = blk[j]
                assert kind == "temporal"
                h = self._temporal(Wb[j], h, g, a["heads"], f"in1.{j}", out=fin(h.shape[0], a["ch"]) if j == last else None)
            first = 2
        for i, blk in enumerate(down_path):
            if i < first:
                continue
            if i == 0 and self.addition_attention:
                h = self._run_block(blk, Wt["in"][i], h, g, f"in{i}")
                h = self._temporal(Wt["init_attn"], h, g, 8, "init_attn", out=skip_dst(0)(h.shape[0], h.shape[1]))
            else:
                h = self._run_block(blk, Wt["in"][i], h, g, f"in{i}", final=skip_dst(i))
        h = self._run_block(middle, Wt["mid"], h, g, "mid", final=lambda rows, cols: cat_view(0, rows, "h"))
        for i, blk in enumerate(up_path):
            ch, cs = self._cat_plan[i]
            if cat_rows.get(i) != h.shape[0]:
                raise ValueError("skip / decoder resolution mismatch (the latent height and width must divide by 8)")
            cat = A.get(f"cat{i}", h.shape[0], ch + cs, device=dev)
            assert h.data_ptr() == cat.data_ptr() and h.shape[1] == ch
            nxt = (lambda rows, cols, u=i + 1: cat_view(u, rows, "h")) if i + 1 < n_up else None
            h = self._run_block(blk, Wt["out"][i], cat, g, f"out{i}", final=nxt)
        n = self._gn(h, Wt["out_gn"], "gn", n_inst=g["F"], rpi=g["HW"], eps=1e-5, silu=True)
        y = A.get("unet_out", h.shape[0], Wt["out_conv"].N, torch.float32, dev)
        conv = dict(IH=g["H"], IW=g["W"], OH=g["H"], OW=g["W"], stride=1, pad=1, ups=0)
        return ops.gemm(n, Wt["out_conv"], y, conv=conv)

    def build_context_rows(self, context, B, T, tag="ctx"):
        dev = context.device
        L, D = context.shape[1], context.shape[2]
        context = context.to(torch.float32).contiguous()
        if L == 77 + T * 16:
            Lc = 77 + 16
            out = self._arena.get(tag, B * T * Lc, D, device=dev)
            ops.build_context(context, out, B=B, T=T, n_text=77, L=16, D=D)
        else:
            Lc = L
            n_text = min(77, L)
            rep = context.repeat_interleave(T, dim=0).contiguous()
            out = self._arena.get(tag, B * T * Lc, D, device=dev)
            ops.build_context(rep, out, B=B * T, T=1, n_text=n_text, L=L - n_text, D=D)
        return out, Lc

    def forward_pair(self, x, cc, timesteps, context, fs=None, **kwargs):
        if not x.is_cuda:
            raise RuntimeError("UNetModel runs on the HIP path only: move the model and inputs to the GPU "
                               "(there is no CPU fallback)")
        B, Cx, T, H, W = x.shape
        Cc = 0 if cc is None else cc.shape[1]
        assert Cx + Cc == self.in_channels
        dev = x.device
        xr = self._arena.get("x_rows", B * T * H * W, C_IN_PAD, device=dev)
        ops.pack_latent(x.to(torch.float32).contiguous(), None if cc is None else cc.to(torch.float32).contiguous(),
                        xr, B=B, Cx=Cx, Cc=Cc, T=T, HW=H * W)
        ctx_rows, Lc = self.build_context_rows(context, B, T)
        t_table = timesteps.to(device=dev, dtype=torch.int64).contiguous()
        if fs is None:
            fs = torch.full((B,), self.default_fs, dtype=torch.int64, device=dev)
        fs_table = fs.to(device=dev, dtype=torch.int64).contiguous()
        y = self.forward_rows(xr, t_table, ctx_rows, B=B, T=T, H=H, W=W, Lc=Lc, n_text=min(77, Lc), fs_table=fs_table)
        out = torch.empty((B, self.out_channels, T, H, W), dtype=torch.float32, device=dev)
        ops.rows_to_nchw(y, out, N=B, Cc=self.out_channels, HW=T * H * W)
        return out

    def forward(self, x, timesteps, context=None, features_adapter=None, fs=None, **kwargs):
        if features_adapter is not None:
            raise NotImplementedError("features_adapter is not part of the DynamiCrafter inference path")
        return self.forward_pair(x, None, timesteps, context, fs=fs)
```

### dynamicrafter_amd/ops.py

```python
import ctypes as C
import os
import math

import torch

from . import _hip
from ._hip import DcDdimParams, DcGemmParams, check

_BF16 = torch.bfloat16


def stream_ptr():
    return C.c_void_p(torch.cuda.current_stream().cuda_stream)


class Tracer:

    def __init__(self):
        self.records = []

    def __enter__(self):
        global _TRACE
        _TRACE = self
        return self

    def __exit__(self, *a):
        global _TRACE
        _TRACE = None

    def _event(self):
        e = C.c_void_p()
        check(_hip.lib().dc_event_create(C.byref(e)), "dc_event_create")
        return e

    def summary(self):
        l = _hip.lib()
        out = {}
        self.detail = {}
        for name, flops, nbytes, e0, e1, tag in self.records:
            ms = C.c_float()
            check(l.dc_event_elapsed_ms(e0, e1, C.byref(ms)), "dc_event_elapsed_ms")
            d = out.setdefault(name, dict(launches=0, ms=0.0, flops=0.0, bytes=0.0))
            d["launches"] += 1; d["ms"] += ms.value; d["flops"] += flops; d["bytes"] += nbytes
            if tag is not None:
                dd = self.detail.setdefault((name, tag), dict(launches=0, ms=0.0, flops=0.0))
                dd["launches"] += 1; dd["ms"] += ms.value; dd["flops"] += flops
            l.dc_event_destroy(e0); l.dc_event_destroy(e1)
        self.records = []
        return out


_TRACE = None


def _launch(name, flops, nbytes, fn, *args, tag=None):
    tr = _TRACE
    if tr is None:
        check(fn(*args), name)
        return
    l = _hip.lib()
    e0, e1 = tr._event(), tr._event()
    sp = stream_ptr()
    l.dc_event_record(e0, sp)
    check(fn(*args), name)
    l.dc_event_record(e1, sp)
    if name == "dc_gemm_conv":
        name = l.dc_gemm_last_variant().decode()
    tr.records.append((name, flops, nbytes, e0, e1, tag))


def _ptr(t):
    return C.c_void_p(0 if t is None else t.data_ptr())


def _rows(t, name="tensor", dtype=_BF16):
    if t.dtype != dtype or t.dim() != 2 or t.stride(1) != 1 or not t.is_cuda:
        raise ValueError(f"{name}: expected CUDA {dtype} rows [R, C] with unit column stride, got "
                         f"{t.dtype} {tuple(t.shape)} strides {t.stride()} on {t.device}")
    return t


class PackedWeight:

    __slots__ = ("w", "bias", "N", "K", "n_pad", "Cin", "taps", "k_real")

    def __init__(self, w, bias, N, K, Cin, taps, k_real=None):
        self.w, self.bias, self.N, self.K, self.Cin, self.taps = w, bias, N, K, Cin, taps
        self.n_pad = w.shape[0]
        self.k_real = k_real

    @staticmethod
    def _finish(w2d, bias, device, Cin, taps, pad_n_to=None):
        N, K = w2d.shape
        n_pad = (N + 127) // 128 * 128
        if pad_n_to is not None:
            n_pad = max(n_pad, pad_n_to)
        wp = torch.zeros((n_pad, K), dtype=_BF16, device=device)
        wp[:N] = w2d.to(device=device, dtype=_BF16)
        b = None if bias is None else bias.detach().to(device=device, dtype=torch.float32).contiguous()
        return PackedWeight(wp, b, N, K, Cin, taps)

    @staticmethod
    def linear(weight, bias, device, n_align=1):
        w = weight.detach().reshape(weight.shape[0], -1)
        N, K = w.shape
        if K % 64 != 0:
            kp = (K + 63) // 64 * 64
            w = torch.nn.functional.pad(w, (0, kp - K))
        if N % n_align != 0:
            npad = (N + n_align - 1) // n_align * n_align
            w = torch.nn.functional.pad(w, (0, 0, 0, npad - N))
            if bias is not None:
                bias = torch.nn.functional.pad(bias.detach(), (0, npad - N))
        return PackedWeight._finish(w, bias, device, w.shape[1], 1)

    @staticmethod
    def conv3x3(weight, bias, device, n_align=1):
        co, ci = weight.shape[0], weight.shape[1]
        w = weight.detach().permute(0, 2, 3, 1)
        cip = (ci + 63) // 64 * 64
        if cip != ci:
            w = torch.nn.functional.pad(w, (0, cip - ci))
        w = w.reshape(co, 9, cip // 64, 64).permute(0, 2, 1, 3).reshape(co, 9 * cip)
        if co % n_align != 0:
            npad = (co + n_align - 1) // n_align * n_align
            w = torch.nn.functional.pad(w, (0, 0, 0, npad - co))
            if bias is not None:
                bias = torch.nn.functional.pad(bias.detach(), (0, npad - co))
        pw = PackedWeight._finish(w, bias, device, cip, 9)
        pw.k_real = 9 * ci
        return pw

    @staticmethod
    def conv3x3_c8_as_linear(weight, bias, device):
        co, ci = weight.shape[0], weight.shape[1]
        assert ci <= 8
        w = torch.zeros(co, 16, 8, dtype=weight.dtype)
        w[:, :9, :ci] = weight.detach().permute(0, 2, 3, 1).reshape(co, 9, ci)
        pw = PackedWeight._finish(w.reshape(co, 128), bias, device, 128, 1)
        pw.k_real = 9 * ci
        return pw

    @staticmethod
    def tconv3(weight, bias, device):
        co, ci = weight.shape[0], weight.shape[1]
        assert ci % 64 == 0, "temporal conv width must be a multiple of 64"
        w = weight.detach().reshape(co, ci // 64, 64, 3).permute(0, 1, 3, 2).reshape(co, 3 * ci)
        return PackedWeight._finish(w, bias, device, ci, 3)


def gemm(a, pw, out, *, M=None, residual=None, rowvec=None, rows_per_vec=1, geglu=False, gelu=False, alpha=1.0,
         conv=None, tconv=None):
    _rows(a, "a")
    out_f32 = out.dtype == torch.float32
    if not out_f32:
        _rows(out, "out")
    p = DcGemmParams()
    p.A, p.W, p.C = a.data_ptr(), pw.w.data_ptr(), out.data_ptr()
    p.bias = 0 if pw.bias is None else pw.bias.data_ptr()
    p.rowvec = 0 if rowvec is None else rowvec.data_ptr()
    p.rowvec_ld = 0 if rowvec is None else rowvec.stride(0)
    p.rows_per_vec = rows_per_vec
    p.residual = 0 if residual is None else _rows(residual, "residual").data_ptr()
    p.ldr = 0 if residual is None else residual.stride(0)
    p.lda, p.ldc = a.stride(0), out.stride(0)
    p.M = out.shape[0] if M is None else M
    p.N, p.K, p.n_pad = pw.N, pw.K, pw.n_pad
    p.Cin = pw.Cin
    p.flags = (_hip.DC_GEMM_OUT_F32 if out_f32 else 0) | (_hip.DC_GEMM_GEGLU if geglu else 0) | \
        (_hip.DC_GEMM_GELU if gelu else 0)
    p.alpha = alpha
    ws = _gemm_workspace(a.device, torch.cuda.current_stream().cuda_stream)
    p.workspace, p.workspace_bytes = ws.data_ptr(), ws.numel()
    if conv is not None:
        p.mode = 1
        p.IH, p.IW, p.OH, p.OW = conv["IH"], conv["IW"], conv["OH"], conv["OW"]
        p.stride, p.pad, p.ups = conv.get("stride", 1), conv.get("pad", 1), conv.get("ups", 0)
        if pw.taps != 9 or a.shape[1] < pw.Cin:
            raise ValueError("conv3x3 weight / activation mismatch")
    elif tconv is not None:
        p.mode = 2
        p.T, p.HW = tconv["T"], tconv["HW"]
        if pw.taps != 3:
            raise ValueError("tconv weight mismatch")
    else:
        p.mode = 0
        if a.shape[1] < pw.K:
            raise ValueError(f"gemm: activation has {a.shape[1]} columns, weight K={pw.K}")
    n_out = pw.N // 2 if geglu else pw.N
    if out.shape[1] < n_out:
        raise ValueError(f"gemm: out has {out.shape[1]} columns, need {n_out}")
    if out.shape[0] < p.M or (residual is not None and (residual.shape[0] < p.M or residual.shape[1] < n_out)):
        raise ValueError(f"gemm: out/residual have fewer than M={p.M} rows (or residual fewer than {n_out} columns)")
    if p.mode == 1:
        if p.M % (p.OH * p.OW) != 0 or a.shape[0] < (p.M // (p.OH * p.OW)) * p.IH * p.IW:
            raise ValueError(f"conv3x3: M={p.M} output rows need {p.M // (p.OH * p.OW)} frames of {p.IH}x{p.IW} input rows, "
                             f"activation has {a.shape[0]}")
    elif a.shape[0] < p.M:
        raise ValueError(f"gemm: activation has {a.shape[0]} rows, M={p.M}")
    if p.mode == 2 and (p.M % (p.T * p.HW) != 0 or a.shape[1] < pw.Cin):
        raise ValueError("tconv: M must be a multiple of T*HW and the activation at least Cin wide")
    if rowvec is not None and (rowvec.shape[0] * rows_per_vec < p.M or rowvec.shape[1] < n_out):
        raise ValueError("gemm: rowvec does not cover every row group / output column")
    if _TRACE is not None:
        variant = "dc_gemm_conv"
        k_real = pw.k_real if pw.k_real else pw.K
        flops = 2.0 * p.M * pw.N * k_real
        esz = 4 if out_f32 else 2
        nbytes = 2.0 * p.M * (k_real if p.mode == 0 else pw.Cin) + 2.0 * pw.N * pw.K + esz * p.M * n_out \
            + (2.0 * p.M * n_out if residual is not None else 0)
        _launch(variant, flops, nbytes, _hip.lib().dc_gemm_conv, C.byref(p), stream_ptr(),
                tag=(p.mode, p.M, pw.N, k_real))
    else:
        check(_hip.lib().dc_gemm_conv(C.byref(p), stream_ptr()), "dc_gemm_conv")
    return out


_gemm_ws = {}


def _gemm_workspace(device, stream):
    key = (device.index, stream)
    buf = _gemm_ws.get(key)
    if buf is None:
        buf = torch.empty(int(_hip.lib().dc_gemm_workspace_bytes()), dtype=torch.uint8, device=device)
        _gemm_ws[key] = buf
    return buf


class Arena:
    GUARD = 8

    def __init__(self):
        self._bufs = {}
        self._guarded = {}
        self.guard = os.environ.get("DC_ARENA_GUARD", "0") == "1"

    def get(self, tag, rows, cols, dtype=_BF16, device=None, zero=False):
        key = (tag, rows, cols, dtype)
        b = self._bufs.get(key)
        if b is None:
            if self.guard:
                G = self.GUARD
                whole = torch.empty((rows + 2 * G, cols), dtype=dtype, device=device)
                whole.fill_(self._sentinel(dtype))
                b = whole[G:G + rows]
                if zero:
                    b.zero_()
                self._guarded[key] = whole
            else:
                b = (torch.zeros if zero else torch.empty)((rows, cols), dtype=dtype, device=device)
            self._bufs[key] = b
        return b

    @staticmethod
    def _sentinel(dtype):
        return 12345.0 if dtype.is_floating_point else 0x5a

    def check(self):
        bad = []
        for (tag, rows, cols, dtype), whole in self._guarded.items():
            G = self.GUARD
            ref = torch.full((1,), self._sentinel(dtype), dtype=dtype, device=whole.device)
            if not (bool((whole[:G] == ref).all()) and bool((whole[G + rows:] == ref).all())):
                bad.append(f"{tag}[{rows}x{cols} {dtype}]")
        if bad:
            raise RuntimeError("scratch buffers overrun: " + ", ".join(bad))
        return len(self._guarded)

    def nbytes(self):
        return sum(b.numel() * b.element_size() for b in self._bufs.values())


_gn_ws = {}


_gn_ws_retired = []


def _gn_workspace(device, nbytes):
    key = (device.index, torch.cuda.current_stream().cuda_stream)
    buf = _gn_ws.get(key)
    if buf is None or buf.numel() * 4 < nbytes:
        if buf is not None:
            _gn_ws_retired.append(buf)
        buf = torch.empty((max(nbytes, 4 << 20) + 3) // 4, dtype=torch.float32, device=device)
        _gn_ws[key] = buf
    return buf


def _need(t, n, name):
    if t is not None and t.numel() < n:
        raise ValueError(f"{name}: {t.numel()} elements, the launch reads/writes {n}")


def _need_rows(t, rows, cols, name):
    if t.shape[0] < rows or t.shape[1] < cols:
        raise ValueError(f"{name}: shape {tuple(t.shape)}, the launch addresses [{rows}, {cols}]")


def groupnorm(x, y, gamma, beta, *, groups, n_inst, rows_per_inst, eps, silu):
    _rows(x, "x"); _rows(y, "y")
    _need_rows(x, n_inst * rows_per_inst, gamma.numel(), "x"); _need_rows(y, n_inst * rows_per_inst, gamma.numel(), "y")
    _need(beta, gamma.numel(), "beta")
    Cc = gamma.numel()
    l = _hip.lib()
    ws = _gn_workspace(x.device, int(l.dc_groupnorm_workspace_bytes(n_inst, groups, rows_per_inst)))
    _launch("groupnorm(2-3 kernels)", 0.0, 6.0 * n_inst * rows_per_inst * Cc, l.dc_groupnorm, _ptr(x), x.stride(0), _ptr(y),
            y.stride(0), _ptr(gamma), _ptr(beta), Cc, groups, n_inst, rows_per_inst, eps, 1 if silu else 0, _ptr(ws),
            stream_ptr())
    return y


def layernorm(x, y, gamma, beta, eps=1e-5):
    _rows(x, "x"); _rows(y, "y")
    _need_rows(x, x.shape[0], gamma.numel(), "x"); _need_rows(y, x.shape[0], gamma.numel(), "y"); _need(beta, gamma.numel(), "beta")
    _launch("layernorm", 0.0, 4.0 * x.shape[0] * gamma.numel(), _hip.lib().dc_layernorm, _ptr(x), x.stride(0), _ptr(y),
            y.stride(0), _ptr(gamma), _ptr(beta), x.shape[0], gamma.numel(), eps, stream_ptr())
    return y


def flash_attn(q, k, v, o, *, batch, heads, Lq, Lk, scale, accumulate=False, acc_scale=1.0, q_bstride=None,
               kv_bstride=None):
    for t, n in ((q, "q"), (k, "k"), (v, "v"), (o, "o")):
        _rows(t, n)
    qb = Lq if q_bstride is None else q_bstride
    kb = Lk if kv_bstride is None else kv_bstride
    _need_rows(q, (batch - 1) * qb + Lq, heads * 64, "q"); _need_rows(o, (batch - 1) * qb + Lq, heads * 64, "o")
    _need_rows(k, (batch - 1) * kb + Lk, heads * 64, "k"); _need_rows(v, (batch - 1) * kb + Lk, heads * 64, "v")
    _launch("flash_attn_d64(self)" if Lk > 128 else "flash_attn_d64(cross)", 4.0 * batch * heads * Lq * Lk * 64,
            2.0 * batch * heads * 64 * (2 * Lq + 2 * Lk), _hip.lib().dc_flash_attn_d64, _ptr(q), _ptr(k), _ptr(v), _ptr(o),
            q.stride(0), k.stride(0), v.stride(0), o.stride(0), batch, heads, Lq, Lk,
            Lq if q_bstride is None else q_bstride, Lk if kv_bstride is None else kv_bstride, scale,
            1 if accumulate else 0, acc_scale, stream_ptr())
    return o


def cross_attn_dual(q, k, v, k2, v2, o, *, batch, heads, Lq, Lk, Lk2, scale, scale2, kv_bstride):
    for t, n in ((q, "q"), (k, "k"), (v, "v"), (k2, "k2"), (v2, "v2"), (o, "o")):
        _rows(t, n)
    if len({k.stride(0), v.stride(0), k2.stride(0), v2.stride(0)}) != 1:
        raise ValueError("cross_attn_dual: k, v, k2, v2 must share one row stride")
    _need_rows(q, batch * Lq, heads * 64, "q"); _need_rows(o, batch * Lq, heads * 64, "o")
    _need_rows(k, (batch - 1) * kv_bstride + Lk, heads * 64, "k"); _need_rows(v, (batch - 1) * kv_bstride + Lk, heads * 64, "v")
    _need_rows(k2, (batch - 1) * kv_bstride + Lk2, heads * 64, "k2"); _need_rows(v2, (batch - 1) * kv_bstride + Lk2, heads * 64, "v2")
    _launch("flash_attn_d64(cross)", 4.0 * batch * heads * Lq * (Lk + Lk2) * 64, 2.0 * batch * heads * 64 * (2 * Lq + 2 * (Lk + Lk2)),
            _hip.lib().dc_cross_attn_dual_d64, _ptr(q), _ptr(k), _ptr(v), _ptr(k2), _ptr(v2), _ptr(o), q.stride(0), k.stride(0),
            o.stride(0), batch, heads, Lq, Lk, Lk2, Lq, kv_bstride, scale, scale2, stream_ptr())
    return o


def temporal_attn(qkv, o, *, B, T, HW, heads, scale):
    _rows(qkv, "qkv"); _rows(o, "o")
    _need_rows(qkv, B * T * HW, 3 * heads * 64, "qkv"); _need_rows(o, B * T * HW, heads * 64, "o")
    _launch("temporal_attn_d64", 4.0 * B * HW * heads * T * T * 64, 2.0 * B * T * HW * heads * 64 * 4,
            _hip.lib().dc_temporal_attn_d64, _ptr(qkv), qkv.stride(0), _ptr(o), o.stride(0), B, T, HW, heads, scale,
            stream_ptr())
    return o


def ff2_permuted(weight, device):
    w = weight.detach()
    N, K = w.shape
    pos = torch.arange(32)
    s_, h_, e_ = pos // 16, (pos // 8) % 2, pos % 8
    chan = 8 * (2 * s_ + e_ // 4) + 4 * h_ + e_ % 4
    idx = (torch.arange(K // 32)[:, None] * 32 + chan[None, :]).reshape(-1)
    n_pad = (N + 127) // 128 * 128
    out = torch.zeros((n_pad, K), dtype=_BF16, device=device)
    out[:N] = w[:, idx].to(device=device, dtype=_BF16)
    return out


def ff_geglu_fused320(x, pw1, w2p, b2, out, residual=None, ln=None, ln_eps=1e-5):
    _rows(x, "x"); _rows(out, "out")
    M = x.shape[0]
    if pw1.K != 320 or pw1.N != 2560 or pw1.bias is None or tuple(w2p.shape[1:]) != (1280,) or w2p.shape[0] < 320:
        raise ValueError("ff_geglu_fused320: dim must be 320 (ff1 [2560, 320] with bias, ff2 [320, 1280])")
    _need_rows(x, M, 320, "x"); _need_rows(out, M, 320, "out")
    if residual is not None:
        _rows(residual, "residual"); _need_rows(residual, M, 320, "residual")
    if ln is not None:
        _need(ln[0], 320, "ln gamma"); _need(ln[1], 320, "ln beta")
    flops = 2.0 * M * (2560 + 1280) * 320
    nbytes = 2.0 * M * 320 * (3 if residual is not None else 2) + 2.0 * (2560 * 320 + 320 * 1280)
    _launch("ff_geglu_fused320", flops, nbytes, _hip.lib().dc_ff_geglu_fused320, _ptr(x), x.stride(0),
            _ptr(None if ln is None else ln[0]), _ptr(None if ln is None else ln[1]), ln_eps, _ptr(pw1.w), _ptr(pw1.bias),
            _ptr(w2p), _ptr(b2), _ptr(residual), 0 if residual is None else residual.stride(0), _ptr(out), out.stride(0), M,
            stream_ptr())
    return out


def ff_geglu_proj_fused320(x, pw1, w2p, b2, wp, bp, residual2, out, ln=None, ln_eps=1e-5):
    _rows(x, "x"); _rows(out, "out"); _rows(residual2, "residual2")
    M = x.shape[0]
    if pw1.K != 320 or pw1.N != 2560 or pw1.bias is None or tuple(w2p.shape[1:]) != (1280,) or w2p.shape[0] < 320 \
            or tuple(wp.shape[1:]) != (320,) or wp.shape[0] < 320:
        raise ValueError("ff_geglu_proj_fused320: dim must be 320 (ff1 [2560, 320] with bias, ff2 [320, 1280], proj [320, 320])")
    if x.data_ptr() == out.data_ptr():
        raise ValueError("ff_geglu_proj_fused320: out must not alias x")
    _need_rows(x, M, 320, "x"); _need_rows(out, M, 320, "out"); _need_rows(residual2, M, 320, "residual2")
    _need(b2, 320, "b2"); _need(bp, 320, "bp")
    if ln is not None:
        _need(ln[0], 320, "ln gamma"); _need(ln[1], 320, "ln beta")
    _launch("ff_geglu_proj_fused320", 2.0 * M * (2560 + 1280 + 320) * 320, 2.0 * M * 320 * 3 + 2.0 * (2560 * 320 + 320 * 1280 + 320 * 320),
            _hip.lib().dc_ff_geglu_proj_fused320, _ptr(x), x.stride(0), _ptr(None if ln is None else ln[0]),
            _ptr(None if ln is None else ln[1]), ln_eps, _ptr(pw1.w), _ptr(pw1.bias), _ptr(w2p), _ptr(b2), _ptr(wp), _ptr(bp),
            _ptr(residual2), residual2.stride(0), _ptr(out), out.stride(0), M, stream_ptr())
    return out


def ln_linear(x, pw, out, ln=None, ln_eps=1e-5):
    _rows(x, "x"); _rows(out, "out")
    M, K = x.shape[0], pw.K
    if K not in (320, 640) or pw.N % 32:
        raise ValueError("ln_linear: K must be 320 or 640 and N a multiple of 32")
    _need_rows(x, M, K, "x"); _need_rows(out, M, pw.N, "out")
    if ln is not None:
        _need(ln[0], K, "ln gamma"); _need(ln[1], K, "ln beta")
    _launch("ln_linear", 2.0 * M * pw.N * K, 2.0 * M * (K + pw.N) + 2.0 * pw.N * K, _hip.lib().dc_ln_linear,
            _ptr(x), x.stride(0), K, _ptr(None if ln is None else ln[0]), _ptr(None if ln is None else ln[1]), ln_eps,
            _ptr(pw.w), _ptr(pw.bias), _ptr(out), out.stride(0), M, pw.N, stream_ptr())
    return out


def linear_residual(x, pw, residual, out):
    _rows(x, "x"); _rows(out, "out"); _rows(residual, "residual")
    M, K = x.shape[0], pw.K
    if K not in (320, 640) or pw.N % 32:
        raise ValueError("linear_residual: K must be 320 or 640 and N a multiple of 32")
    _need_rows(x, M, K, "x"); _need_rows(out, M, pw.N, "out"); _need_rows(residual, M, pw.N, "residual")
    _launch("linear_residual", 2.0 * M * pw.N * K, 2.0 * M * (K + 2 * pw.N) + 2.0 * pw.N * K, _hip.lib().dc_linear_residual,
            _ptr(x), x.stride(0), K, _ptr(pw.w), _ptr(pw.bias), _ptr(residual), residual.stride(0), _ptr(out), out.stride(0),
            M, pw.N, stream_ptr())
    return out


def ln_qkv_temporal_attn(x, ln, pw_qkv, out, *, B, T, HW, scale, ln_eps=1e-5):
    _rows(x, "x"); _rows(out, "out")
    M = B * T * HW
    Cc = pw_qkv.K
    if Cc not in (320, 640) or pw_qkv.N != 3 * Cc or pw_qkv.bias is not None or T != 16 or HW % 8:
        raise ValueError("ln_qkv_temporal_attn: dim 320 / 640 (qkv weight [3 C, C], no bias), T = 16, HW % 8 == 0")
    if x.data_ptr() == out.data_ptr():
        raise ValueError("ln_qkv_temporal_attn: out must not alias x")
    _need_rows(x, M, Cc, "x"); _need_rows(out, M, Cc, "out"); _need(ln[0], Cc, "ln gamma"); _need(ln[1], Cc, "ln beta")
    fn = _hip.lib().dc_ln_qkv_temporal_attn320 if Cc == 320 else _hip.lib().dc_ln_qkv_temporal_attn640
    _launch(f"ln_qkv_temporal_attn{Cc}", 2.0 * M * 3 * Cc * Cc + 4.0 * M * T * Cc, 4.0 * M * Cc + 2.0 * 3 * Cc * Cc,
            fn, _ptr(x), x.stride(0), _ptr(ln[0]), _ptr(ln[1]), ln_eps, _ptr(pw_qkv.w),
            _ptr(out), out.stride(0), B, T, HW, scale, stream_ptr())
    return out


def ln_qkv_temporal_attn320(x, ln, pw_qkv, out, *, B, T, HW, scale, ln_eps=1e-5):
    if pw_qkv.K != 320:
        raise ValueError("ln_qkv_temporal_attn320: dim 320 (qkv weight [960, 320], no bias), T = 16, HW % 8 == 0")
    return ln_qkv_temporal_attn(x, ln, pw_qkv, out, B=B, T=T, HW=HW, scale=scale, ln_eps=ln_eps)


def gn_silu_tconv3(x, gamma, beta, stats, pw, out, *, B, T, HW, groups=32, residual=None):
    _rows(x, "x"); _rows(out, "out")
    M = B * T * HW
    C = pw.w.shape[1] // 3
    if C not in (320, 640) or pw.w.shape[1] != 3 * C or pw.N % 32 or pw.bias is None or T != 16 or HW % 8:
        raise ValueError("gn_silu_tconv3: 320 / 640 input channels (weight [N, 3 C] with bias), N % 32 == 0, T = 16, HW % 8 == 0")
    if x.data_ptr() == out.data_ptr():
        raise ValueError("gn_silu_tconv3: out must not alias x")
    _need_rows(x, M, C, "x"); _need_rows(out, M, pw.N, "out")
    _need(gamma, C, "gamma"); _need(beta, C, "beta"); _need(stats, B * groups * 2, "stats")
    if residual is not None:
        _rows(residual, "residual"); _need_rows(residual, M, pw.N, "residual")
    _launch("gn_silu_tconv3", 2.0 * M * pw.N * 3 * C, 2.0 * M * (C + pw.N * (2 if residual is not None else 1)) + 2.0 * pw.N * 3 * C,
            _hip.lib().dc_gn_silu_tconv3, _ptr(x), x.stride(0), C, _ptr(gamma), _ptr(beta), _ptr(stats), groups, _ptr(pw.w),
            _ptr(pw.bias), _ptr(residual), 0 if residual is None else residual.stride(0), _ptr(out), out.stride(0), B, T, HW,
            pw.N, stream_ptr())
    return out


def groupnorm_stats(x, stats, *, groups, n_inst, rows_per_inst, eps):
    _rows(x, "x")
    Cc = x.shape[1]
    _need_rows(x, n_inst * rows_per_inst, Cc, "x"); _need(stats, n_inst * groups * 2, "stats")
    l = _hip.lib()
    ws = _gn_workspace(x.device, int(l.dc_groupnorm_workspace_bytes(n_inst, groups, rows_per_inst)))
    _launch("groupnorm_stats(2 kernels)", 0.0, 2.0 * n_inst * rows_per_inst * Cc, l.dc_groupnorm_stats, _ptr(x), x.stride(0),
            Cc, groups, n_inst, rows_per_inst, eps, _ptr(ws), _ptr(stats), stream_ptr())
    return stats


def gn_linear(x, gamma, beta, stats, pw, out, *, groups, rows_per_inst):
    _rows(x, "x"); _rows(out, "out")
    M, K = x.shape[0], pw.K
    if K not in (320, 640) or pw.N % 32 or rows_per_inst % 128 or M % rows_per_inst:
        raise ValueError("gn_linear: K in (320, 640), N % 32 == 0, rows_per_inst % 128 == 0, M % rows_per_inst == 0")
    _need_rows(x, M, K, "x"); _need_rows(out, M, pw.N, "out")
    _need(gamma, K, "gamma"); _need(beta, K, "beta"); _need(stats, (M // rows_per_inst) * groups * 2, "stats")
    _launch("gn_linear", 2.0 * M * pw.N * K, 2.0 * M * (K + pw.N) + 2.0 * pw.N * K, _hip.lib().dc_gn_linear,
            _ptr(x), x.stride(0), K, _ptr(gamma), _ptr(beta), _ptr(stats), groups, rows_per_inst, _ptr(pw.w), _ptr(pw.bias),
            _ptr(out), out.stride(0), M, pw.N, stream_ptr())
    return out


def attn_small(q, k, v, o, *, batch, heads, Lq, Lk, d, scale, causal=False):
    for t, n in ((q, "q"), (k, "k"), (v, "v"), (o, "o")):
        _rows(t, n)
    _need_rows(q, batch * Lq, heads * d, "q"); _need_rows(o, batch * Lq, heads * d, "o")
    _need_rows(k, batch * Lk, heads * d, "k"); _need_rows(v, batch * Lk, heads * d, "v")
    _launch("attn_small", 4.0 * batch * heads * Lq * Lk * d, 2.0 * batch * heads * d * (2 * Lq + 2 * Lk),
            _hip.lib().dc_attn_small, _ptr(q), _ptr(k), _ptr(v), _ptr(o), q.stride(0), k.stride(0), v.stride(0), o.stride(0),
            batch, heads, Lq, Lk, d, scale, 1 if causal else 0, stream_ptr())
    return o

# ... 321 lines not shown
```

### include/dcrafter_hip.h

```cpp
#ifndef DCRAFTER_HIP_H
#define DCRAFTER_HIP_H
#include <stdint.h>

#ifdef __cplusplus
extern "C" {
#endif

#define DC_ERR_SHAPE (-1)
#define DC_ERR_ARG   (-2)

#define DC_GEMM_OUT_F32 1
#define DC_GEMM_GEGLU   2
#define DC_GEMM_GELU    4

typedef struct DcGemmParams {
    const uint16_t* A;
    const uint16_t* W;
    void* C;
    const float* bias;
    const float* rowvec;
    const uint16_t* residual;
    int lda, ldc, ldr, rowvec_ld;
    int rows_per_vec;
    int M, N, K, n_pad;
    int mode;
    int Cin;
    int IH, IW, OH, OW;
    int stride, pad, ups;
    int T, HW;
    int flags;
    float alpha;
    void* workspace;
    long long workspace_bytes;
} DcGemmParams;

const char* dc_gemm_last_variant(void);

int dc_gemm_set_plan(int plan);

int64_t dc_gemm_workspace_bytes(void);

int dc_gemm_conv(const DcGemmParams* p, void* stream);

int dc_groupnorm(const uint16_t* x, int ldx, uint16_t* y, int ldy, const float* gamma, const float* beta,
                 int C, int groups, int n_inst, int rows_per_inst, float eps, int silu,
                 float* workspace, void* stream);
int64_t dc_groupnorm_workspace_bytes(int n_inst, int groups, int rows_per_inst);

int dc_layernorm(const uint16_t* x, int ldx, uint16_t* y, int ldy, const float* gamma, const float* beta,
                 int rows, int C, float eps, void* stream);

int dc_flash_attn_d64(const uint16_t* q, const uint16_t* k, const uint16_t* v, uint16_t* o,
                      int ldq, int ldk, int ldv, int ldo, int batch, int heads, int Lq, int Lk,
                      int64_t q_bstride, int64_t kv_bstride, float scale, int accumulate, float acc_scale,
                      void* stream);

int dc_flash_attn_set_mode(int mode, float thr);

int dc_temporal_attn_d64(const uint16_t* qkv, int ld, uint16_t* o, int ldo, int B, int T, int HW, int heads,
                         float scale, void* stream);

int dc_gemv_small(const float* in, int ld_in, const uint16_t* W, const float* bias, float* out, int ld_out,
                  int M, int N, int K, int act_in, int act_out, int accumulate, void* stream);

int dc_timestep_embedding(const int64_t* t_table, const int32_t* t_index, int t_stride, float* out, int B, int dim,
                          float max_period, void* stream);

int dc_pack_latent(const float* x, const float* cc, uint16_t* out, int B, int Cx, int Cc, int T, int HW,
                   int c_pad, int nrep, void* stream);

int dc_nchw_to_rows(const float* x, uint16_t* out, int N, int C, int HW, int c_pad, float scale, void* stream);
int dc_rows_to_nchw(const void* rows, int ld, int rows_f32, float* y, int N, int C, int HW, float scale, void* stream);

int dc_im2col3x3_c8(const uint16_t* x, int ldx, uint16_t* out, int ldo, int n_img, int H, int W, void* stream);

int dc_copy2d(const uint16_t* src, int lds, uint16_t* dst, int ldd, int rows, int cols, void* stream);

int dc_build_context(const float* ctx, uint16_t* out, int B, int T, int n_text, int L, int D, void* stream);

int dc_softmax_rows(const float* x, int ldx, uint16_t* y, int ldy, int rows, int cols, void* stream);

int dc_transpose(const uint16_t* src, int lds, uint16_t* dst, int ldd, int rows, int cols, void* stream);

int dc_add_rows(const uint16_t* a, int lda, const uint16_t* b, int ldb, uint16_t* y, int ldy, int rows, int cols,
                void* stream);

int dc_vae_sample(const uint16_t* moments, int ld, const float* noise, float* z, int N, int zc, int HW,
                  float scale, void* stream);

typedef struct DcDdimParams {
    const float* a_t;
    const float* a_prev;
    const float* sigma_t;
    const float* sqrt_one_minus_at;
    const float* sqrt_acp_t;
    const float* sqrt_1macp_t;
    const float* scale_ratio;
    const int32_t* step_index;
    int index;
    int v_param;
    float cfg_scale;
    float cfg_img;
    float guidance_rescale;
    float temperature;
    int e_nchw;
    int64_t noise_step_stride;
} DcDdimParams;

int dc_ddim_step(const DcDdimParams* p, const float* e_cond, const float* e_uncond, const float* e_img, int ld_e,
                 const float* x, const float* noise, float* x_prev, float* pred_x0, int B, int C, int THW,
                 float* workspace, void* stream);

typedef struct DcDpmParams {
    const float* A;
    const float* alpha_t;
    const float* alpha_p_r;
    const float* k;
    const float* N;
    const float* sqrt_one_minus_at;
    const float* sqrt_acp_t;
    const float* sqrt_1macp_t;
    const float* scale_ratio;
    const int32_t* step_index;
    int index;
    int v_param;
    float cfg_scale;
    float cfg_img;
    float guidance_rescale;
    float temperature;
    int e_nchw;
    int64_t noise_step_stride;
    float* x0_hist;
} DcDpmParams;

int dc_dpmpp_step(const DcDpmParams* p, const float* e_cond, const float* e_uncond, const float* e_img, int ld_e,
                  const float* x, const float* noise, float* x_prev, float* pred_x0, int B, int C, int THW,
                  float* workspace, void* stream);

typedef struct DcSdsParams {
    const float* c1;
    const float* c2;
    const float* w;
    const float* step_size;
    const float* bc2_sqrt;
    const int32_t* step_index;
    int index;
    int weight_type;
    int x0_param;
    int e_nchw;
    float cfg_scale;
    float guidance_rescale;
    float beta2, eps;
    float one_minus_beta1;
    float one_minus_beta2;
    float decay;
    float grad_scale;
    int64_t noise_step_stride;
    float* loss;
} DcSdsParams;

int dc_sds_noise(const DcSdsParams* p, const float* latent, const float* noise, float* x_t, int B, int64_t n_per_clip,
                 void* stream);

int dc_sds_step(const DcSdsParams* p, const float* e_cond, const float* e_uncond, int ld_e, const float* x_t,
                float* latent, float* m, float* v, int B, int C, int THW, float* workspace, void* stream);

int dc_cross_attn_dual_d64(const uint16_t* q, const uint16_t* k, const uint16_t* v, const uint16_t* k2, const uint16_t* v2,
                           uint16_t* o, int ldq, int ldkv, int ldo, int batch, int heads, int Lq, int Lk, int Lk2,
                           int64_t q_bstride, int64_t kv_bstride, float scale, float scale2, void* stream);

int dc_ff_geglu_fused320(const uint16_t* x, int ldx, const float* ln_gamma, const float* ln_beta, float ln_eps,
                         const uint16_t* w1, const float* b1, const uint16_t* w2p, const float* b2, const uint16_t* residual,
                         int ldr, uint16_t* out, int ldo, int M, void* stream);

int dc_ff_geglu_proj_fused320(const uint16_t* x, int ldx, const float* ln_gamma, const float* ln_beta, float ln_eps,
                              const uint16_t* w1, const float* b1, const uint16_t* w2p, const float* b2, const uint16_t* wp,
                              const float* bp, const uint16_t* residual2, int ldr2, uint16_t* out, int ldo, int M, void* stream);

int dc_ln_linear(const uint16_t* x, int ldx, int K, const float* ln_gamma, const float* ln_beta, float ln_eps, const uint16_t* w,
                 const float* bias, uint16_t* out, int ldo, int M, int N, void* stream);
int dc_groupnorm_stats(const uint16_t* x, int ldx, int C, int groups, int n_inst, int rows_per_inst, float eps,
                       float* workspace, float* stats_out, void* stream);
int dc_gn_linear(const uint16_t* x, int ldx, int K, const float* gamma, const float* beta, const float* stats, int groups,
                 int rows_per_inst, const uint16_t* w, const float* bias, uint16_t* out, int ldo, int M, int N, void* stream);

int dc_linear_residual(const uint16_t* x, int ldx, int K, const uint16_t* w, const float* bias, const uint16_t* residual, int ldr,
                       uint16_t* out, int ldo, int M, int N, void* stream);

int dc_ln_qkv_temporal_attn320(const uint16_t* x, int ldx, const float* ln_gamma, const float* ln_beta, float ln_eps,
                               const uint16_t* wqkv, uint16_t* out, int ldo, int B, int T, int HW, float scale, void* stream);
int dc_ln_qkv_temporal_attn640(const uint16_t* x, int ldx, const float* ln_gamma, const float* ln_beta, float ln_eps,
                               const uint16_t* wqkv, uint16_t* out, int ldo, int B, int T, int HW, float scale, void* stream);

int dc_gn_silu_tconv3(const uint16_t* x, int ldx, int C, const float* gamma, const float* beta, const float* stats, int groups,
                      const uint16_t* w, const float* bias, const uint16_t* residual, int ldr, uint16_t* out, int ldo, int B, int T,
                      int HW, int N, void* stream);


int dc_attn_small(const uint16_t* q, const uint16_t* k, const uint16_t* v, uint16_t* o, int ldq, int ldk, int ldv, int ldo,
                  int B, int heads, int Lq, int Lk, int d, float scale, int causal, void* stream);
int64_t dc_attn_small_lds_bytes(int Lk, int d);

int dc_clip_preprocess(const float* img, float* tmp0, float* tmp1, float* out, int N, int C, int H, int W, int OH, int OW,
                       int antialias, const float* mean3, const float* std3, void* stream);

int dc_patchify(const float* img, uint16_t* rows, int N, int C, int H, int W, int p, int kpad, void* stream);

int dc_embed_tokens(const int64_t* tokens, const uint16_t* table, const uint16_t* pos, uint16_t* out, int B, int L, int D,
                    int vocab, void* stream);

int dc_frames_to_u8(const float* video, uint8_t* out, int N, int C, int T, int H, int W, void* stream);

int dc_mask_blend(float* img, const float* x0, const float* mask, const float* qnoise, const float* sqrt_acp_t,
                  const float* sqrt_1macp_t, const int32_t* step_index, int index, int64_t n,
                  int64_t noise_step_stride, int clean, void* stream);

int dc_advance_counter(int32_t* counter, void* stream);

int dc_stream_create(void** stream_out);
int dc_stream_destroy(void* stream);
int dc_stream_sync(void* stream);
int dc_graph_begin_capture(void* stream);
int dc_graph_end_capture(void* stream, void** graph_exec_out);
int dc_graph_launch(void* graph_exec, void* stream);
int dc_graph_destroy(void* graph_exec);
int dc_event_create(void** ev_out);
int dc_event_record(void* ev, void* stream);
int dc_event_elapsed_ms(void* ev_start, void* ev_stop, float* ms_out);
int dc_event_destroy(void* ev);

int dc_error_word_read(int* out, int reset);

const char* dc_version(void);

#ifdef __cplusplus
}
#endif
#endif
```

Before: 2.592 frames/s.

## Fold resblock 1x1 skip into conv2 K-loop and batch all timestep-embedding GEMVs

Adds a second K segment to the pipelined 320-wide conv GEMM kernel, so a ResBlock's 1x1 skip projection can be computed as extra K columns of conv2 ([W | Wskip] weight, second A operand). This removes a separate skip GEMM and its output round trip, but the fold is off by default (DC_RES_SKIP_FOLD=0). Separately, all ResBlock emb_layers linears are concatenated into one weight and evaluated with a single gemv per step, which is on by default and replaces many tiny launches. The fold path only handles a narrow set of shapes and falls back to the plain weights otherwise.

```diff
diff --git a/dynamicrafter_amd/_hip.py b/dynamicrafter_amd/_hip.py
--- a/dynamicrafter_amd/_hip.py
+++ b/dynamicrafter_amd/_hip.py
@@ -23,6 +23,7 @@
         ("T", C.c_int), ("HW", C.c_int),
         ("flags", C.c_int), ("alpha", C.c_float),
         ("workspace", C.c_void_p), ("workspace_bytes", C.c_longlong),
+        ("A2", C.c_void_p), ("lda2", C.c_int), ("K2", C.c_int),
     ]
 
 
@@ -63,6 +64,7 @@
 _P, _I, _F, _L = C.c_void_p, C.c_int, C.c_float, C.c_int64
 SIGNATURES = {
     "dc_gemm_conv": (_I, [C.POINTER(DcGemmParams), _P]),
+    "dc_gemm_k2_ok": (_I, [C.POINTER(DcGemmParams)]),
     "dc_gemm_workspace_bytes": (_L, []),
     "dc_gemm_last_variant": (C.c_char_p, []),
     "dc_gemm_set_plan": (_I, [_I]),
diff --git a/dynamicrafter_amd/csrc/gemm_conv.hip b/dynamicrafter_amd/csrc/gemm_conv.hip
--- a/dynamicrafter_amd/csrc/gemm_conv.hip
+++ b/dynamicrafter_amd/csrc/gemm_conv.hip
@@ -554,6 +554,7 @@
 }
 
 int dc_gemm_conv_glds_try(const DcGemmParams& p, hipStream_t stream);
+bool dc_gemm_k2_accept(const DcGemmParams& p);
 
 static bool glds_enabled() {
     static int v = -1;
@@ -572,10 +573,19 @@
     return (int64_t)8 * 40 * 256 * 320 * 4;
 }
 
+extern "C" int dc_gemm_k2_ok(const DcGemmParams* pp) {
+    return (pp && pp->K2 > 0 && glds_enabled() && dc_gemm_k2_accept(*pp)) ? 1 : 0;
+}
+
 extern "C" int dc_gemm_conv(const DcGemmParams* pp, void* stream_) {
     const DcGemmParams& p = *pp;
     hipStream_t stream = (hipStream_t)stream_;
     if (p.M <= 0 || p.N <= 0 || p.K <= 0) return DC_ERR_SHAPE;
+    if (p.K2 != 0) {
+        if (!dc_gemm_k2_ok(pp)) return DC_ERR_ARG;
+        const int r = dc_gemm_conv_glds_try(p, stream);
+        return r == -100 ? DC_ERR_ARG : r;
+    }
     if (p.K % BK != 0 || p.N % 4 != 0 || p.lda % 8 != 0 || p.ldc % 4 != 0) return DC_ERR_SHAPE;
     if (p.mode != 0 && (p.Cin % BK != 0)) return DC_ERR_SHAPE;
     if (p.mode == 1 && p.K != 9 * p.Cin) return DC_ERR_SHAPE;
diff --git a/dynamicrafter_amd/csrc/gemm_conv_glds.hip b/dynamicrafter_amd/csrc/gemm_conv_glds.hip
--- a/dynamicrafter_amd/csrc/gemm_conv_glds.hip
+++ b/dynamicrafter_amd/csrc/gemm_conv_glds.hip
@@ -852,6 +852,10 @@
 int launch_pipe_shape(const DcGemmParams& p, hipStream_t stream, GemmSplit sp, int gx, int gy) {
     sp.err = dc_error_word_device();
     if (!sp.err) return DC_ERR_ARG;
+    if (p.K2 > 0) {
+        if constexpr (MODE == 1) return launch_pipe320x16<1, EPI, true>(p, stream, sp, gx, gy);
+        else return DC_ERR_ARG;
+    }
     return launch_pipe320x16<MODE, EPI>(p, stream, sp, gx, gy);
 }
 
@@ -861,10 +865,14 @@
     if (p.flags & (DC_GEMM_GEGLU | DC_GEMM_OUT_F32)) return false;
     if (p.ups && !(p.mode == 1 && p.ups == 1 && p.stride == 1 && p.pad == 1 && p.OH == 2 * p.IH && p.OW == 2 * p.IW)) return false;
     if (p.N % 320 != 0 || p.n_pad < p.N || p.K % 64 != 0 || p.lda % 8 != 0 || ((uintptr_t)p.A % 16) != 0) return false;
+    if (p.K2 != 0) {
+        if (p.K2 < 0 || p.K2 % 64 != 0 || !p.A2 || p.mode != 1 || p.ups || p.stride != 1 || p.pad != 1 || p.OH != p.IH || p.OW != p.IW || p.OH <= 0 || p.OW <= 0) return false;
+        if (p.lda2 < p.K2 || p.lda2 % 8 != 0 || ((uintptr_t)p.A2 % 16) != 0 || (long long)p.M * p.lda2 * 2 >= (1ll << 31)) return false;
+    }
     if (p.ldc % 8 != 0 || ((uintptr_t)p.C % 16) != 0 || (long long)p.M * p.ldc >= (1ll << 31)) return false;
     if (p.residual && (p.ldr % 8 != 0 || ((uintptr_t)p.residual % 16) != 0 || (long long)p.M * p.ldr >= (1ll << 31))) return false;
     long long rows = p.M, extra = 0;
-    if (p.mode == 1) { if (p.Cin % 64 != 0 || p.K != 9 * p.Cin) return false; rows = (long long)(p.M / (p.OH * p.OW) + 1) * p.IH * p.IW; extra = 2ll * p.IW + 2; }
+    if (p.mode == 1) { if (p.Cin <= 0 || p.Cin % 64 != 0 || p.K != 9 * p.Cin + p.K2) return false; rows = (long long)(p.M / (p.OH * p.OW) + 1) * p.IH * p.IW; extra = 2ll * p.IW + 2; }
     else if (p.mode == 2) { if (p.Cin % 64 != 0 || p.K != 3 * p.Cin) return false; extra = 2ll * p.HW; }
     else if (p.mode != 0) return false;
     if ((rows + extra) * p.lda * 2 >= (1ll << 31)) return false;
@@ -877,7 +885,7 @@
     GemmSplit sp;
     sp.partial = nullptr; sp.splits = 1; sp.tile_begin = 0; sp.tile_count = ntiles; sp.err = nullptr; sp.whole = 0;
     dc_note_variant(p.mode == 0 ? "gemm_pipe320x16_kernel" : p.mode == 2 ? "gemm_pipe320x16_kernel<tconv>"
-                    : p.ups ? "gemm_pipe320x16_kernel<conv,ups>" : "gemm_pipe320x16_kernel<conv>");
+                    : p.ups ? "gemm_pipe320x16_kernel<conv,ups>" : p.K2 ? "gemm_pipe320x16_kernel<conv+k2>" : "gemm_pipe320x16_kernel<conv>");
     if (p.mode == 0) return p.residual ? launch_pipe_shape<0, 1>(p, stream, sp, ntiles, 1) : launch_pipe_shape<0, 0>(p, stream, sp, ntiles, 1);
     if (p.mode == 1 && p.ups) return p.residual ? launch_pipe_shape<3, 1>(p, stream, sp, ntiles, 1) : launch_pipe_shape<3, 0>(p, stream, sp, ntiles, 1);
     if (p.mode == 1) return p.residual ? launch_pipe_shape<1, 1>(p, stream, sp, ntiles, 1) : launch_pipe_shape<1, 0>(p, stream, sp, ntiles, 1);
@@ -893,7 +901,8 @@
     if constexpr (BN == 320) {
         if (use_pipe) {
             dc_note_variant(MODE == 0 ? "gemm_pipe320x16_kernel+splitk" : MODE == 2 ? "gemm_pipe320x16_kernel<tconv>+splitk"
-                            : MODE == 3 ? "gemm_pipe320x16_kernel<conv,ups>+splitk" : "gemm_pipe320x16_kernel<conv>+splitk");
+                            : MODE == 3 ? "gemm_pipe320x16_kernel<conv,ups>+splitk"
+                            : p.K2 ? "gemm_pipe320x16_kernel<conv+k2>+splitk" : "gemm_pipe320x16_kernel<conv>+splitk");
             GemmSplit sp;
             sp.err = nullptr; sp.whole = 0;
             if (full > 0 && merged && full % 8 == 0) {
@@ -941,6 +950,14 @@
     return launch_glds<BN, false, 2, GSTAGES>(p, stream);
 }
 
+inline int force_tile() { static const int v = [] { const char* e = getenv("DC_GEMM_TILE"); return e ? atoi(e) : 0; }(); return v; }
+inline bool k2_accept(const DcGemmParams& p, int plan) {
+    if (p.K2 <= 0 || p.M <= 0 || p.N <= 0 || p.K <= p.K2 || !p.A || !p.W || !p.C || ((uintptr_t)p.W % 16) != 0) return false;
+    if (force_tile() != 0 || !pipe_ok(p, plan)) return false;
+    if (p.M % (p.OH * p.OW) != 0) return false;
+    return (long long)((p.M + GBM - 1) / GBM) * (p.N / 320) >= 8;
+}
+
 inline int persist_max_k() {
     static const int v = [] { const char* e = getenv("DC_GEMM_PERSIST_MAXK"); return e ? atoi(e) : 2560; }();
     return v;
@@ -954,7 +971,7 @@
     const bool geglu = (p.flags & DC_GEMM_GEGLU) != 0;
     const int n_out = geglu ? p.N / 2 : p.N;
     const int tiles_m = (p.M + GBM - 1) / GBM;
-    static const int force = [] { const char* e = getenv("DC_GEMM_TILE"); return e ? atoi(e) : 0; }();
+    const int force = force_tile();
     static const int persist = [] { const char* e = getenv("DC_GEMM_PERSIST"); return e ? atoi(e) : 1; }();
     if (geglu && p.mode != 0) return DC_ERR_ARG;
     const bool out_f32 = (p.flags & DC_GEMM_OUT_F32) != 0;
@@ -963,6 +980,7 @@
                                    (!p.residual || ((p.ldr % 8 == 0) && ((uintptr_t)p.residual % 16 == 0))));
     const int plan = g_gemm_plan.load(std::memory_order_relaxed);
     const bool use_pipe = pipe_ok(p, plan);
+    if (p.K2 != 0 && !k2_accept(p, plan)) return DC_ERR_ARG;
     const bool prefer_pipe = (force == 0) && use_pipe;
     if (persist && force == 0 && p.mode == 0 && epi16 && p.K <= persist_max_k() && !prefer_pipe) {
         static const int wide = [] { const char* e = getenv("DC_GEMM_PERSIST_WIDE"); return e ? atoi(e) : 1; }();
@@ -1042,6 +1060,7 @@
             }
         }
     }
+    if (p.K2 != 0) return launch_pipe_whole(p, stream);
     if (force == 320 && n320) return use_pipe ? launch_pipe_whole(p, stream) : launch_glds_mode<320, 2>(p, stream);
     if (force == 128 && w128 > 0 && waste128 <= 1.15f) return launch_glds_mode<128, 3>(p, stream);
     if (force == 1) return -100;
@@ -1054,6 +1073,8 @@
 
 int dc_gemm_plan_now() { return g_gemm_plan.load(std::memory_order_relaxed); }
 
+bool dc_gemm_k2_accept(const DcGemmParams& p) { return k2_accept(p, g_gemm_plan.load(std::memory_order_relaxed)); }
+
 extern "C" int dc_gemm_set_plan(int plan) {
     if (!plan_valid(plan)) return DC_ERR_ARG;
     return g_gemm_plan.exchange(plan & PLAN_MASK, std::memory_order_relaxed);
diff --git a/dynamicrafter_amd/csrc/gemm_pipe16.h b/dynamicrafter_amd/csrc/gemm_pipe16.h
--- a/dynamicrafter_amd/csrc/gemm_pipe16.h
+++ b/dynamicrafter_amd/csrc/gemm_pipe16.h
@@ -16,7 +16,7 @@
     asm volatile("s_nop 7\n\ts_nop 7" ::: "memory");
 }
 
-template <int MODE, int EPI>
+template <int MODE, int EPI, bool SEG2 = false>
 __global__ __launch_bounds__(256, 1) __attribute__((amdgpu_waves_per_eu(1, 1)))
 void gemm_pipe320x16_kernel(const DcGemmParams p, const GemmSplit sp) {
     extern __shared__ __attribute__((aligned(16))) char smem[];
@@ -117,11 +117,42 @@
         ars[2] = 0x7fffffff;
         ars[3] = 0x00020000;
     }
+    static_assert(!SEG2 || MODE == 1, "the second K segment rides the plain 3x3 conv only");
+    const int nk1 = SEG2 ? (p.K - p.K2) / GBK : 0;
+    unsigned rowoff2[4];
+    int ars2_lo = 0, ars2_hi = 0;
+    if constexpr (SEG2) {
+#pragma unroll
+        for (int rb = 0; rb < 4; ++rb) {
+            const int m = m0 + wave * 64 + rb * 16 + lr_a;
+            rowoff2[rb] = m < p.M ? (unsigned)m * ((unsigned)p.lda2 * 2u) + lq_a * 16 : 0x80000000u;
+        }
+        const unsigned long long ab2 = (unsigned long long)(uintptr_t)p.A2;
+        ars2_lo = __builtin_amdgcn_readfirstlane((int)(unsigned)ab2);
+        ars2_hi = __builtin_amdgcn_readfirstlane((int)(unsigned)((ab2 >> 32) & 0xffffu));
+    }
+    auto a_desc = [&](int kt) __attribute__((always_inline)) -> gp_i32x4_t {
+        gp_i32x4_t rs = ars;
+        if constexpr (SEG2) {
+            const bool seg = __builtin_amdgcn_readfirstlane(kt >= nk1 ? 1 : 0) != 0;
+            rs[0] = seg ? ars2_lo : ars[0];
+            rs[1] = seg ? ars2_hi : ars[1];
+        }
+        return rs;
+    };
     auto a_tile = [&](int kt, unsigned (&vo)[4], int& soff) __attribute__((always_inline)) {
         int tap = 0;
         if (MODE == 0) {
             soff = kt * 128;
         } else if (MODE == 1) {
+            if constexpr (SEG2) {
+                if (kt >= nk1) {
+                    soff = (kt - nk1) * 128;
+#pragma unroll
+                    for (int rb = 0; rb < 4; ++rb) vo[rb] = rowoff2[rb];
+                    return;
+                }
+            }
             const int cs = kt / 9;
             tap = kt - cs * 9;
             const int dy = tap / 3, dx = tap - dy * 3;
@@ -194,10 +225,11 @@
         unsigned vo[4];
         int soff;
         a_tile(clampk(t), vo, soff);
+        const gp_i32x4_t rs = a_desc(clampk(t));
 #pragma unroll
         for (int i = 0; i < 8; ++i) {
-            if ((i >> 2) == 0) GP_LOAD_A_(A[t][i & 3][0], vo[i & 3], ars, soff, "0");
-            else GP_LOAD_A_(A[t][i & 3][1], vo[i & 3], ars, soff, "64");
+            if ((i >> 2) == 0) GP_LOAD_A_(A[t][i & 3][0], vo[i & 3], rs, soff, "0");
+            else GP_LOAD_A_(A[t][i & 3][1], vo[i & 3], rs, soff, "64");
         }
     }
     wait_vmcnt<26>();
@@ -218,6 +250,7 @@
         unsigned vo[4] = {0u, 0u, 0u, 0u};
         int soff = 0;
         unsigned long long ws = 0;
+        gp_i32x4_t rs = ars;
         gp_f32x4_t (&acc1)[4][20] = acc;
         bf16x8_t (&Bf1)[5] = Bf;
         u32x4_t (&A1)[3][4][2] = A;
@@ -255,11 +288,12 @@
 #endif
                         __hip_atomic_fetch_add(cnt_landed, 1, __ATOMIC_RELAXED, __HIP_MEMORY_SCOPE_WORKGROUP);
                     a_tile(kt2, vo, soff);
+                    rs = a_desc(kt2);
                 }
                 if constexpr (g >= 90 && g <= 146 && ((g - 90) & 7) == 0) {
                     constexpr int i = (g - 90) >> 3;
-                    if constexpr ((i >> 2) == 0) GP_LOAD_A_(A_[ST2][i & 3][0], vo[i & 3], ars, soff, "0");
-                    else GP_LOAD_A_(A_[ST2][i & 3][1], vo[i & 3], ars, soff, "64");
+                    if constexpr ((i >> 2) == 0) GP_LOAD_A_(A_[ST2][i & 3][0], vo[i & 3], rs, soff, "0");
+                    else GP_LOAD_A_(A_[ST2][i & 3][1], vo[i & 3], rs, soff, "64");
                 }
                 if constexpr (g == 118) seen_l = *(volatile gp_lds_int_t*)cnt_landed;
                 if constexpr (g == 142) {
@@ -361,11 +395,11 @@
     }
 }
 
-template <int MODE, int EPI>
+template <int MODE, int EPI, bool SEG2 = false>
 int launch_pipe320x16(const DcGemmParams& p, hipStream_t stream, const GemmSplit& sp, int grid_x, int grid_y) {
     static DcLdsOnce lds_once;
-    if (const int e = lds_once.ensure(reinterpret_cast<const void*>(&gemm_pipe320x16_kernel<MODE, EPI>), GP_LDS)) return e;
-    hipLaunchKernelGGL((gemm_pipe320x16_kernel<MODE, EPI>), dim3(grid_x, grid_y), dim3(256), GP_LDS, stream, p, sp);
+    if (const int e = lds_once.ensure(reinterpret_cast<const void*>(&gemm_pipe320x16_kernel<MODE, EPI, SEG2>), GP_LDS)) return e;
+    hipLaunchKernelGGL((gemm_pipe320x16_kernel<MODE, EPI, SEG2>), dim3(grid_x, grid_y), dim3(256), GP_LDS, stream, p, sp);
     DC_CHECK_LAUNCH();
     return 0;
 }
diff --git a/dynamicrafter_amd/lvdm/modules/networks/openaimodel3d.py b/dynamicrafter_amd/lvdm/modules/networks/openaimodel3d.py
--- a/dynamicrafter_amd/lvdm/modules/networks/openaimodel3d.py
+++ b/dynamicrafter_amd/lvdm/modules/networks/openaimodel3d.py
@@ -17,6 +17,8 @@
 _TA_FUSED_C = tuple(int(k) for k in os.environ.get("DC_TA_FUSED_C", "320,640").split(","))
 _FFP_FUSED = os.environ.get("DC_FFP_FUSED", "1") != "0"
 _TC_FUSED = os.environ.get("DC_TC_FUSED", "1") != "0"
+_RES_SKIP_FOLD = os.environ.get("DC_RES_SKIP_FOLD", "0") != "0"
+_EMB_BATCHED = os.environ.get("DC_EMB_BATCHED", "1") != "0"
 _FUSED_MIN_ROWS = int(os.environ.get("DC_FUSED_MIN_ROWS", "4096"))
 _LN_FUSED_K = tuple(int(k) for k in os.environ.get("DC_LN_FUSED_K", "320,640").split(","))
 C_IN_PAD = 64
@@ -310,11 +312,14 @@
                 elif kind == "res":
                     d = {"gn1": (f32(p + ".in_layers.0.weight"), f32(p + ".in_layers.0.bias")),
                          "conv1": PackedWeight.conv3x3(self._p(p + ".in_layers.2.weight"), self._p(p + ".in_layers.2.bias"), device),
-                         "emb": lin(p + ".emb_layers.1"),
                          "gn2": (f32(p + ".out_layers.0.weight"), f32(p + ".out_layers.0.bias")),
-                         "conv2": PackedWeight.conv3x3(self._p(p + ".out_layers.3.weight"), self._p(p + ".out_layers.3.bias"), device)}
-                    if a["cin"] != a["cout"]:
-                        d["skip"] = lin(p + ".skip_connection")
+                         "name": p}
+                    if a["cin"] != a["cout"] and _RES_SKIP_FOLD and a["cout"] % 320 == 0 and a["cin"] % 64 == 0:
+                        d["conv2_skip"] = PackedWeight.conv3x3_skip1x1(
+                            self._p(p + ".out_layers.3.weight"), self._p(p + ".out_layers.3.bias"),
+                            self._p(p + ".skip_connection.weight"), self._p(p + ".skip_connection.bias"), device)
+                    else:
+                        self._res_plain_weights(d, device)
                     if a["tconv"]:
                         d["tc"] = []
                         for i, ci in ((1, 2), (2, 3), (3, 3), (4, 3)):
@@ -337,6 +342,16 @@
         P["in"] = [pack_block(f"input_blocks.{i}", b) for i, b in enumerate(down_path)]
         P["mid"] = pack_block("middle_block", middle)
         P["out"] = [pack_block(f"output_blocks.{i}", b) for i, b in enumerate(up_path)]
+        res = [d for grp in P["in"] + [P["mid"]] + P["out"] for d in grp if "gn1" in d]
+        names = [d["name"] + ".emb_layers.1" for d in res]
+        P["emb_all"] = PackedWeight.linear(torch.cat([self._p(n + ".weight").detach() for n in names], 0),
+                                           torch.cat([self._p(n + ".bias").detach() for n in names], 0), device)
+        off = 0
+        for d in res:
+            n = d["conv1"].N
+            d["emb_off"] = off
+            d["emb"] = PackedWeight(P["emb_all"].w[off:off + n], P["emb_all"].bias[off:off + n], n, P["emb_all"].K, P["emb_all"].K, 1)
+            off += n
         P["out_gn"] = (f32("out.0.weight"), f32("out.0.bias"))
         P["out_conv"] = PackedWeight.conv3x3(self._p("out.2.weight"), self._p("out.2.bias"), device, n_align=4)
         P["device"] = device
@@ -357,24 +372,46 @@
         y = self._arena.get(tag, x.shape[0], x.shape[1], device=x.device)
         return ops.layernorm(x, y, wb[0], wb[1], 1e-5)
 
+    def _res_plain_weights(self, W, device):
+        p = W["name"]
+        if "conv2" not in W:
+            W["conv2"] = PackedWeight.conv3x3(self._p(p + ".out_layers.3.weight"), self._p(p + ".out_layers.3.bias"), device)
+            if self._has(p + ".skip_connection.weight"):
+                W["skip"] = PackedWeight.linear(self._p(p + ".skip_connection.weight"), self._p(p + ".skip_connection.bias"), device)
+        return W
+
+    def _res_fold_ok(self, W, h, x, dst, conv):
+        key = (h.shape[0], h.stride(0), x.stride(0), dst.stride(0), conv["IH"], conv["IW"])
+        ok = W.setdefault("fold_ok", {}).get(key)
+        if ok is None:
+            ok = W["fold_ok"][key] = ops.gemm_k2_ok(h, W["conv2_skip"], dst, conv=conv, a2=x)
+        return ok
+
     def _res(self, W, x, g, out_tag, out=None):
         A = self._arena
         M, dev = x.shape[0], x.device
         cout = W["conv1"].N
         conv = dict(IH=g["H"], IW=g["W"], OH=g["H"], OW=g["W"], stride=1, pad=1, ups=0)
-        emb_out = A.get("emb_out", g["B"], cout, torch.float32, dev)
-        ops.gemv_small(g["emb"], W["emb"], emb_out, act_in=1)
+        if g.get("emb_all") is not None:
+            emb_out = g["emb_all"][:g["B"], W["emb_off"]:W["emb_off"] + cout]
+        else:
+            emb_out = A.get("emb_out", g["B"], cout, torch.float32, dev)
+            ops.gemv_small(g["emb"], W["emb"], emb_out, act_in=1)
         h = self._gn(x, W["gn1"], "gn", n_inst=g["F"], rpi=g["HW"], eps=1e-5, silu=True)
         h1 = ops.gemm(h, W["conv1"], A.get("res_h1", M, cout, device=dev), conv=conv, rowvec=emb_out,
                       rows_per_vec=g["T"] * g["HW"])
         h = self._gn(h1, W["gn2"], "gn", n_inst=g["F"], rpi=g["HW"], eps=1e-5, silu=True)
-        skip = x
-        if "skip" in W:
-            skip = ops.gemm(x, W["skip"], A.get("res_skip", M, cout, device=dev))
         has_tc = "tc" in W
         final = (lambda: out if out is not None else A.get(out_tag, M, cout, device=dev))
-        h2 = ops.gemm(h, W["conv2"], A.get("res_h2", M, cout, device=dev) if has_tc else final(), conv=conv,
-                      residual=skip)
+        dst = A.get("res_h2", M, cout, device=dev) if has_tc else final()
+        if "conv2_skip" in W and self._res_fold_ok(W, h, x, dst, conv):
+            h2 = ops.gemm(h, W["conv2_skip"], dst, conv=conv, a2=x)
+        else:
+            self._res_plain_weights(W, dev)
+            skip = x
+            if "skip" in W:
+                skip = ops.gemm(x, W["skip"], A.get("res_skip", M, cout, device=dev))
+            h2 = ops.gemm(h, W["conv2"], dst, conv=conv, residual=skip)
         if not has_tc:
             return h2
         tc = dict(T=g["T"], HW=g["HW"])
@@ -562,7 +599,11 @@
             ops.gemv_small(hid, Wt["fps2"], emb, accumulate=True)
         if ctx_kv is not None and ctx_kv.get("__gen__") != Wt["gen"]:
             ctx_kv = None
-        g = dict(B=B, T=T, F=B * T, H=H, W=W, HW=H * W, emb=emb, ctx=ctx_rows, Lc=Lc, n_text=n_text, ctx_kv=ctx_kv)
+        emb_all = None
+        if _EMB_BATCHED:
+            emb_all = A.get("emb_all", B, Wt["emb_all"].N, torch.float32, dev)
+            ops.gemv_small(emb, Wt["emb_all"], emb_all, act_in=1)
+        g = dict(B=B, T=T, F=B * T, H=H, W=W, HW=H * W, emb=emb, emb_all=emb_all, ctx=ctx_rows, Lc=Lc, n_text=n_text, ctx_kv=ctx_kv)
         down_path, middle, up_path = self._layout
         n_up = len(up_path)
 
diff --git a/dynamicrafter_amd/ops.py b/dynamicrafter_amd/ops.py
--- a/dynamicrafter_amd/ops.py
+++ b/dynamicrafter_amd/ops.py
@@ -82,12 +82,13 @@
 
 class PackedWeight:
 
-    __slots__ = ("w", "bias", "N", "K", "n_pad", "Cin", "taps", "k_real")
+    __slots__ = ("w", "bias", "N", "K", "n_pad", "Cin", "taps", "k_real", "k2")
 
     def __init__(self, w, bias, N, K, Cin, taps, k_real=None):
         self.w, self.bias, self.N, self.K, self.Cin, self.taps = w, bias, N, K, Cin, taps
         self.n_pad = w.shape[0]
         self.k_real = k_real
+        self.k2 = 0
 
     @staticmethod
     def _finish(w2d, bias, device, Cin, taps, pad_n_to=None):
@@ -132,6 +133,27 @@
         return pw
 
     @staticmethod
+    def conv3x3_skip1x1(weight, bias, skip_weight, skip_bias, device):
+        co, ci = weight.shape[0], weight.shape[1]
+        assert ci % 64 == 0 and skip_weight.shape[0] == co
+        w = weight.detach().permute(0, 2, 3, 1).reshape(co, 9, ci // 64, 64).permute(0, 2, 1, 3).reshape(co, 9 * ci)
+        ws = skip_weight.detach().reshape(co, -1)
+        cs = ws.shape[1]
+        k2 = (cs + 63) // 64 * 64
+        if k2 != cs:
+            ws = torch.nn.functional.pad(ws, (0, k2 - cs))
+        b = None
+        if bias is not None or skip_bias is not None:
+            b = torch.zeros(co, dtype=torch.float32)
+            for t in (bias, skip_bias):
+                if t is not None:
+                    b = b + t.detach().to(device="cpu", dtype=torch.float32)
+        pw = PackedWeight._finish(torch.cat([w, ws.to(w.dtype)], dim=1), b, device, ci, 9)
+        pw.k2 = k2
+        pw.k_real = 9 * ci + cs
+        return pw
+
+    @staticmethod
     def conv3x3_c8_as_linear(weight, bias, device):
         co, ci = weight.shape[0], weight.shape[1]
         assert ci <= 8
@@ -149,8 +171,8 @@
         return PackedWeight._finish(w, bias, device, ci, 3)
 
 
-def gemm(a, pw, out, *, M=None, residual=None, rowvec=None, rows_per_vec=1, geglu=False, gelu=False, alpha=1.0,
-         conv=None, tconv=None):
+def _gemm_params(a, pw, out, *, M=None, residual=None, rowvec=None, rows_per_vec=1, geglu=False, gelu=False, alpha=1.0,
+                 conv=None, tconv=None, a2=None):
     _rows(a, "a")
     out_f32 = out.dtype == torch.float32
     if not out_f32:
@@ -202,12 +224,32 @@
         raise ValueError("tconv: M must be a multiple of T*HW and the activation at least Cin wide")
     if rowvec is not None and (rowvec.shape[0] * rows_per_vec < p.M or rowvec.shape[1] < n_out):
         raise ValueError("gemm: rowvec does not cover every row group / output column")
+    if (a2 is not None) != (pw.k2 > 0):
+        raise ValueError("gemm: a second operand goes with a [W | W2] weight (PackedWeight.conv3x3_skip1x1), and only with one")
+    if a2 is not None:
+        _rows(a2, "a2")
+        if p.mode != 1 or a2.shape[0] < p.M or a2.shape[1] < pw.k2:
+            raise ValueError(f"gemm: a2 must hold M={p.M} rows of {pw.k2} columns for a 3x3 conv, got {tuple(a2.shape)}")
+        p.A2, p.lda2, p.K2 = a2.data_ptr(), a2.stride(0), pw.k2
+    return p, n_out
+
+
+def gemm_k2_ok(a, pw, out, **kw):
+    p, _ = _gemm_params(a, pw, out, **kw)
+    return bool(_hip.lib().dc_gemm_k2_ok(C.byref(p)))
+
+
+def gemm(a, pw, out, *, M=None, residual=None, rowvec=None, rows_per_vec=1, geglu=False, gelu=False, alpha=1.0,
+         conv=None, tconv=None, a2=None):
+    p, n_out = _gemm_params(a, pw, out, M=M, residual=residual, rowvec=rowvec, rows_per_vec=rows_per_vec, geglu=geglu, gelu=gelu,
+                            alpha=alpha, conv=conv, tconv=tconv, a2=a2)
+    out_f32 = out.dtype == torch.float32
     if _TRACE is not None:
         variant = "dc_gemm_conv"
         k_real = pw.k_real if pw.k_real else pw.K
         flops = 2.0 * p.M * pw.N * k_real
         esz = 4 if out_f32 else 2
-        nbytes = 2.0 * p.M * (k_real if p.mode == 0 else pw.Cin) + 2.0 * pw.N * pw.K + esz * p.M * n_out \
+        nbytes = 2.0 * p.M * (k_real if p.mode == 0 else pw.Cin + pw.k2) + 2.0 * pw.N * pw.K + esz * p.M * n_out \
             + (2.0 * p.M * n_out if residual is not None else 0)
         _launch(variant, flops, nbytes, _hip.lib().dc_gemm_conv, C.byref(p), stream_ptr(),
                 tag=(p.mode, p.M, pw.N, k_real))
diff --git a/include/dcrafter_hip.h b/include/dcrafter_hip.h
--- a/include/dcrafter_hip.h
+++ b/include/dcrafter_hip.h
@@ -32,6 +32,9 @@
     float alpha;
     void* workspace;
     long long workspace_bytes;
+    const uint16_t* A2;
+    int lda2;
+    int K2;
 } DcGemmParams;
 
 const char* dc_gemm_last_variant(void);
@@ -41,6 +44,8 @@
 int64_t dc_gemm_workspace_bytes(void);
 
 int dc_gemm_conv(const DcGemmParams* p, void* stream);
+
+int dc_gemm_k2_ok(const DcGemmParams* p);
 
 int dc_groupnorm(const uint16_t* x, int ldx, uint16_t* y, int ldy, const float* gamma, const float* beta,
                  int C, int groups, int n_inst, int rows_per_inst, float eps, int silu,
```

After: 2.599 frames/s, median of 6. About the same (+0.3%).
